# Enhex/RGK

Hardware: AMD Instinct MI355X
Metric: Mpaths/s, Sponza 1920x1080x256spp (path-tracing hot path) (higher is better)
Workload: dtype f32; 1 GPU; sponza-1080p 1920x1080x256spp depth 2 russian 0.74, strong scaling; geometry=proxy, triangles=64536, sampler=halton-cp, textures=handed over as u8; 0 of 0 float textures stored as bytes + value table, tiles=2040, parallelism=tiles round-robin over 1 GPU(s) + one RCCL reduce per round

## Files before the change

include/rgk.h:

```cpp
#ifndef RGK_H
#define RGK_H

#include <stdint.h>

#ifdef __cplusplus
extern "C" {
#endif

typedef enum rgk_status {
    RGK_OK = 0,
    RGK_ERR_INVALID = -1,
    RGK_ERR_DEVICE = -2,
    RGK_ERR_OOM = -3,
    RGK_ERR_NO_DEVICE = -4,
    RGK_ERR_UNSUPPORTED = -5
} rgk_status;

typedef enum rgk_bxdf_kind {
    RGK_BXDF_DIFFUSE = 0,
    RGK_BXDF_MIRROR = 1,
    RGK_BXDF_DIELECTRIC = 2,
    RGK_BXDF_TRANSPARENT = 3,
    RGK_BXDF_MIX = 4,
    RGK_BXDF_LTC_BECKMANN = 5,
// ... 97 lines not shown
typedef enum rgk_sampler_kind {
    RGK_SAMPLER_HALTON = 0,
    RGK_SAMPLER_STRATIFIED = 1
} rgk_sampler_kind;

#define RGK_FLAG_COUNT_TRAVERSAL 1u
#define RGK_FLAG_TIME_KERNELS 2u

typedef struct rgk_params {
    uint32_t xres, yres;
    uint32_t multisample;
    uint32_t depth;
    float clamp;
    float russian;
    float bumpmap_scale;
    uint32_t force_fresnell;
    uint32_t reverse;
    uint32_t sampler;
    uint32_t flags;
} rgk_params;

typedef struct rgk_tile {
    uint32_t x0, x1, y0, y1;
    uint32_t seed;
} rgk_tile;

typedef enum rgk_kernel_id {
    RGK_K_TRACE_CAMERA = 0,
    RGK_K_TRACE_CLOSEST,
    RGK_K_SHADE_FIRST,
    RGK_K_SHADE,
    RGK_K_SHADOW_FIRST,
    RGK_K_SHADOW,
    RGK_K_SHADOW_JOBS,
    RGK_K_CONNECT,
    RGK_K_LIGHT_TRACE,
    RGK_K_LIGHT_SHADE,
    RGK_K_LIGHT_SPLAT,
    RGK_K_RESOLVE,
    RGK_K_OTHER,
    RGK_K_COUNT
} rgk_kernel_id;

typedef struct rgk_kernel_stat {
    double ms;
    uint32_t launches;
    uint32_t reserved;
    uint64_t units;
    uint64_t node_visits;
    uint64_t tri_tests;
} rgk_kernel_stat;

typedef struct rgk_counters {
    uint64_t paths;
    uint64_t path_rays;
    uint64_t shadow_rays;
    uint64_t node_visits;
    uint64_t tri_tests;
    uint64_t shadow_node_visits;
    uint64_t shadow_tri_tests;
    double ms_trace;
    double ms_shadow;
    double ms_shade;
    double ms_other;
    uint32_t n_trace_launches;
    uint32_t n_shadow_launches;
    uint32_t n_shade_launches;
    uint32_t reserved;
    rgk_kernel_stat kernel[RGK_K_COUNT];
} rgk_counters;

typedef struct rgk_scene_info {
    float epsilon;
    float bbox_min[3];
    float bbox_max[3];
    float total_areal_power, total_point_power;
    uint32_t n_nodes;
    uint32_t node_bytes;
    uint32_t tri_bytes;
    uint32_t max_depth;
    uint32_t n_leaf_refs;
    uint32_t n_float_textures;
    uint32_t n_palettized_textures;
} rgk_scene_info;

typedef struct rgk_hit {
    float t;
    int32_t tri;
    float a, b, c;
} rgk_hit;

typedef struct rgk_progress {
    uint32_t stage, stages;
    uint32_t rounds;
    uint32_t busy;
    uint64_t round_pixels;
    uint64_t round_paths;
} rgk_progress;

typedef struct rgk_scene rgk_scene;

const char *rgk_last_error(void);
int rgk_device_count(void);

int rgk_scene_create(const rgk_scene_desc *desc, int device, rgk_scene **out);
int rgk_scene_refit(rgk_scene *scene, const float *vertices, const float *normals, const float *tangents);
void rgk_scene_destroy(rgk_scene *scene);
int rgk_scene_get_info(const rgk_scene *scene, rgk_scene_info *out);

int rgk_scene_get_progress(const rgk_scene *scene, rgk_progress *out);

int rgk_scene_set_tuning(rgk_scene *scene, const char *key, double value);

int rgk_generate_task_list(uint32_t tile_size, uint32_t xres, uint32_t yres, float mid_x,
                           float mid_y, uint32_t seedstart, uint32_t seedcount_base,
                           rgk_tile *tiles, uint32_t *n_tiles);

int rgk_camera_init(rgk_camera *out, const float pos[3], const float lookat[3], const float up[3], float yview,
                    float xview, int32_t xsize, int32_t ysize, float focus_plane, float lens_size);

int rgk_render_round(rgk_scene *scene, const rgk_camera *camera, const rgk_params *params,
                     const rgk_tile *tiles, uint32_t n_tiles, float *accum_rgb,
                     uint32_t *accum_count, rgk_counters *counters);

int rgk_render_round_device(rgk_scene *scene, const rgk_camera *camera,
                            const rgk_params *params, const rgk_tile *tiles, uint32_t n_tiles,
                            float *d_accum_rgb, uint32_t *d_accum_count,
                            rgk_counters *counters);

typedef struct rgk_accum rgk_accum;
int rgk_accum_create(uint32_t xres, uint32_t yres, int device, rgk_accum **out);
void rgk_accum_destroy(rgk_accum *acc);
int rgk_accum_clear(rgk_accum *acc);
float *rgk_accum_rgb(rgk_accum *acc);
uint32_t *rgk_accum_count(rgk_accum *acc);
int rgk_accum_download(const rgk_accum *acc, float *rgb, uint32_t *count);
int rgk_accum_upload(rgk_accum *acc, const float *rgb, const uint32_t *count);
int rgk_accum_add(rgk_accum *dst, const rgk_accum *src);
int rgk_accum_set_tag(rgk_accum *acc, uint64_t tag);

int rgk_accum_save(const rgk_accum *acc, const char *path, uint32_t rounds_done, uint32_t seedcount);
int rgk_accum_load(rgk_accum *acc, const char *path, uint32_t *rounds_done, uint32_t *seedcount);

typedef struct rgk_comm rgk_comm;
#define RGK_COMM_ID_BYTES 128
int rgk_shard_tiles(const rgk_tile *tiles, uint32_t n_tiles, int rank, int world_size, rgk_tile *out, uint32_t *n_out);
int rgk_comm_get_unique_id(uint8_t id[RGK_COMM_ID_BYTES]);
int rgk_comm_create(const uint8_t id[RGK_COMM_ID_BYTES], int rank, int world_size, int device, rgk_comm **out);
void rgk_comm_destroy(rgk_comm *comm);
int rgk_accum_reduce(rgk_comm *comm, float *d_accum_rgb, uint32_t *d_accum_count, uint32_t xres, uint32_t yres, int root);

int rgk_trace_closest(rgk_scene *scene, uint32_t n, const float *rays, const int32_t *ignore,
                      rgk_hit *hits, rgk_counters *counters);

int rgk_trace_visibility(rgk_scene *scene, uint32_t n, const float *a, const float *b,
                         uint8_t *visible, rgk_counters *counters);

int rgk_bxdf_value(rgk_scene *scene, uint32_t n, uint32_t route, const uint32_t *mat, const float *Vi, const float *Vr,
                   const float *uv, float *out_rgb);
int rgk_bxdf_sample(rgk_scene *scene, uint32_t n, uint32_t route, const uint32_t *mat, const float *Vi, const float *uv,
                    const float *u, float *out_dir, float *out_weight, uint8_t *may_leak);
int rgk_texture_sample(rgk_scene *scene, uint32_t n, const int32_t *tex, const float *uv, float *rgb, float *slope_right,
                       float *slope_bottom);

int rgk_libm_eval(int fn, uint32_t n, const float *a, const float *b, float *out);

// ... 16 lines not shown
```

rgk_amd/capi.py:

```python
import ctypes as C
import os

HERE = os.path.dirname(os.path.abspath(__file__))
LIB_PATH = os.environ.get("RGK_LIB") or os.path.join(HERE, "csrc", "librgk_hip.so")

BXDF_DIFFUSE, BXDF_MIRROR, BXDF_DIELECTRIC, BXDF_TRANSPARENT, BXDF_MIX = 0, 1, 2, 3, 4
BXDF_LTC_BECKMANN, BXDF_LTC_GGX, BXDF_LTC_BECKMANN_DIFFUSE, BXDF_LTC_GGX_DIFFUSE = 5, 6, 7, 8
MAT_NO_RUSSIAN = 1
TEX_SOLID, TEX_RGB32F, TEX_RGB8 = 0, 1, 2
SKY_COLOR, SKY_ENVMAP = 0, 1
SAMPLER_HALTON, SAMPLER_STRATIFIED = 0, 1
FLAG_COUNT_TRAVERSAL, FLAG_TIME_KERNELS = 1, 2
BUILD_AUTO, BUILD_DEVICE, BUILD_KEEP_FLOAT_TEXTURES, BUILD_HOST_SAH = 0, 1, 2, 4

BRDF_IDS = {
    "diffusecosine": BXDF_DIFFUSE, "diffuse": BXDF_DIFFUSE, "mix": BXDF_MIX,
    "dielectric": BXDF_DIELECTRIC, "mirror": BXDF_MIRROR, "transparent": BXDF_TRANSPARENT,
    "ltc_beckmann": BXDF_LTC_BECKMANN, "ltc_ggx": BXDF_LTC_GGX,
    "ltc_beckmann_diffuse": BXDF_LTC_BECKMANN_DIFFUSE, "ltc_ggx_diffuse": BXDF_LTC_GGX_DIFFUSE,
}

f3 = C.c_float * 3


class Material(C.Structure):
    _fields_ = [("kind", C.c_uint32), ("flags", C.c_uint32), ("emission", f3),
                ("roughness", C.c_float), ("ior", C.c_float), ("amount", C.c_float),
                ("tex_diffuse", C.c_int32), ("tex_color", C.c_int32), ("tex_bump", C.c_int32),
                ("mix_m1", C.c_int32), ("mix_m2", C.c_int32)]


class Texture(C.Structure):
    _fields_ = [("kind", C.c_uint32), ("width", C.c_uint32), ("height", C.c_uint32),
                ("color", f3), ("texels", C.POINTER(C.c_float)), ("texels8", C.POINTER(C.c_uint8)),
                ("lut", C.POINTER(C.c_float))]


class PointLight(C.Structure):
    _fields_ = [("pos", f3), ("color", f3), ("intensity", C.c_float), ("size", C.c_float)]


class SceneDesc(C.Structure):
    _fields_ = [("n_vertices", C.c_uint32),
                ("vertices", C.POINTER(C.c_float)), ("normals", C.POINTER(C.c_float)),
                ("tangents", C.POINTER(C.c_float)), ("texcoords", C.POINTER(C.c_float)),
                ("n_triangles", C.c_uint32),
                ("tri_indices", C.POINTER(C.c_uint32)), ("tri_material", C.POINTER(C.c_uint32)),
                ("n_materials", C.c_uint32), ("materials", C.POINTER(Material)),
                ("n_textures", C.c_uint32), ("textures", C.POINTER(Texture)),
                ("n_pointlights", C.c_uint32), ("pointlights", C.POINTER(PointLight)),
                ("n_areal_lights", C.c_uint32),
                ("areal_offsets", C.POINTER(C.c_uint32)), ("areal_tris", C.POINTER(C.c_uint32)),
                ("sky_mode", C.c_uint32), ("sky_color", f3), ("sky_intensity", C.c_float),
                ("sky_rotate", C.c_float), ("sky_texture", C.c_int32),
                ("ltc_ggx", C.POINTER(C.c_float)), ("ltc_beckmann", C.POINTER(C.c_float)), ("build_flags", C.c_uint32)]


class Camera(C.Structure):
    _fields_ = [("origin", f3), ("direction", f3), ("cameraup", f3), ("cameraleft", f3),
                ("viewscreen", f3), ("viewscreen_x", f3), ("viewscreen_y", f3),
                ("lens_size", C.c_float), ("xsize", C.c_int32), ("ysize", C.c_int32)]


class Params(C.Structure):
    _fields_ = [("xres", C.c_uint32), ("yres", C.c_uint32), ("multisample", C.c_uint32),
                ("depth", C.c_uint32), ("clamp", C.c_float), ("russian", C.c_float),
                ("bumpmap_scale", C.c_float), ("force_fresnell", C.c_uint32),
                ("reverse", C.c_uint32), ("sampler", C.c_uint32), ("flags", C.c_uint32)]


class Tile(C.Structure):
    _fields_ = [("x0", C.c_uint32), ("x1", C.c_uint32), ("y0", C.c_uint32), ("y1", C.c_uint32),
                ("seed", C.c_uint32)]


KERNEL_IDS = ["trace_camera", "trace_closest", "shade_first", "shade", "shadow_first", "shadow", "shadow_jobs", "connect",
              "light_trace", "light_shade", "light_splat", "resolve", "other"]
KERNEL_NAMES = {"trace_camera": "k_trace_camera", "trace_closest": "k_trace_closest", "shade_first": "k_shade<false, true", "shade": "k_shade<false, false",
                "shadow_first": "k_trace_shadow_first", "shadow": "k_trace_shadow<", "shadow_jobs": "k_trace_shadow_jobs", "connect": "k_connect",
                "resolve": "k_resolve"}


class KernelStat(C.Structure):
    _fields_ = [("ms", C.c_double), ("launches", C.c_uint32), ("reserved", C.c_uint32), ("units", C.c_uint64),
                ("node_visits", C.c_uint64), ("tri_tests", C.c_uint64)]


class Counters(C.Structure):
    _fields_ = [("paths", C.c_uint64), ("path_rays", C.c_uint64), ("shadow_rays", C.c_uint64),
                ("node_visits", C.c_uint64), ("tri_tests", C.c_uint64),
                ("shadow_node_visits", C.c_uint64), ("shadow_tri_tests", C.c_uint64),
                ("ms_trace", C.c_double), ("ms_shadow", C.c_double), ("ms_shade", C.c_double),
                ("ms_other", C.c_double), ("n_trace_launches", C.c_uint32),
                ("n_shadow_launches", C.c_uint32), ("n_shade_launches", C.c_uint32),
                ("reserved", C.c_uint32), ("kernel", KernelStat * len(KERNEL_IDS))]

    def as_dict(self):
        return {k: getattr(self, k) for k, _ in self._fields_ if k not in ("reserved", "kernel")}


class SceneInfo(C.Structure):
    _fields_ = [("epsilon", C.c_float), ("bbox_min", f3), ("bbox_max", f3),
                ("total_areal_power", C.c_float), ("total_point_power", C.c_float),
                ("n_nodes", C.c_uint32), ("node_bytes", C.c_uint32), ("tri_bytes", C.c_uint32),
                ("max_depth", C.c_uint32), ("n_leaf_refs", C.c_uint32),
                ("n_float_textures", C.c_uint32), ("n_palettized_textures", C.c_uint32)]


class Progress(C.Structure):
    _fields_ = [("stage", C.c_uint32), ("stages", C.c_uint32), ("rounds", C.c_uint32), ("busy", C.c_uint32),
                ("round_pixels", C.c_uint64), ("round_paths", C.c_uint64)]


class Hit(C.Structure):
    _fields_ = [("t", C.c_float), ("tri", C.c_int32), ("a", C.c_float), ("b", C.c_float),
                ("c", C.c_float)]


EXPORTS = ["rgk_last_error", "rgk_device_count", "rgk_scene_create", "rgk_scene_destroy",
           "rgk_scene_get_info", "rgk_scene_get_progress", "rgk_scene_set_tuning", "rgk_scene_refit", "rgk_generate_task_list", "rgk_camera_init", "rgk_render_round",
           "rgk_render_round_device", "rgk_trace_closest", "rgk_trace_visibility",
           "rgk_bxdf_value", "rgk_bxdf_sample", "rgk_texture_sample",
           "rgk_libm_eval", "rgk_sampler_eval", "rgk_output_normalize", "rgk_output_write_exr", "rgk_float_to_half",
           "rgk_accum_create", "rgk_accum_destroy", "rgk_accum_clear", "rgk_accum_rgb", "rgk_accum_count",
           "rgk_accum_download", "rgk_accum_upload", "rgk_accum_add", "rgk_accum_set_tag", "rgk_accum_save", "rgk_accum_load",
           "rgk_shard_tiles", "rgk_comm_get_unique_id", "rgk_comm_create", "rgk_comm_destroy", "rgk_accum_reduce"]

_p = C.POINTER


def _bind(lib):
    lib.rgk_last_error.restype = C.c_char_p
    lib.rgk_device_count.restype = C.c_int
    lib.rgk_scene_create.argtypes = [_p(SceneDesc), C.c_int, _p(C.c_void_p)]
    lib.rgk_scene_destroy.argtypes = [C.c_void_p]
    lib.rgk_scene_destroy.restype = None
    lib.rgk_scene_get_info.argtypes = [C.c_void_p, _p(SceneInfo)]
    lib.rgk_scene_get_progress.argtypes = [C.c_void_p, _p(Progress)]
    lib.rgk_scene_set_tuning.argtypes = [C.c_void_p, C.c_char_p, C.c_double]
    lib.rgk_scene_refit.argtypes = [C.c_void_p, C.c_void_p, C.c_void_p, C.c_void_p]
    lib.rgk_generate_task_list.argtypes = [C.c_uint32, C.c_uint32, C.c_uint32, C.c_float, C.c_float,
                                           C.c_uint32, C.c_uint32, _p(Tile), _p(C.c_uint32)]
    lib.rgk_camera_init.argtypes = [_p(Camera), f3, f3, f3, C.c_float, C.c_float, C.c_int32, C.c_int32, C.c_float, C.c_float]
    lib.rgk_render_round.argtypes = [C.c_void_p, _p(Camera), _p(Params), _p(Tile), C.c_uint32,
                                     C.c_void_p, C.c_void_p, _p(Counters)]
    lib.rgk_render_round_device.argtypes = lib.rgk_render_round.argtypes
    lib.rgk_trace_closest.argtypes = [C.c_void_p, C.c_uint32, C.c_void_p, C.c_void_p, C.c_void_p,
                                      _p(Counters)]
    lib.rgk_trace_visibility.argtypes = [C.c_void_p, C.c_uint32, C.c_void_p, C.c_void_p,
                                         C.c_void_p, _p(Counters)]
    lib.rgk_bxdf_value.argtypes = [C.c_void_p, C.c_uint32, C.c_uint32, C.c_void_p, C.c_void_p, C.c_void_p, C.c_void_p, C.c_void_p]
    lib.rgk_bxdf_sample.argtypes = [C.c_void_p, C.c_uint32, C.c_uint32, C.c_void_p, C.c_void_p, C.c_void_p, C.c_void_p, C.c_void_p, C.c_void_p, C.c_void_p]
    lib.rgk_texture_sample.argtypes = [C.c_void_p, C.c_uint32, C.c_void_p, C.c_void_p, C.c_void_p, C.c_void_p, C.c_void_p]
    lib.rgk_libm_eval.argtypes = [C.c_int, C.c_uint32, C.c_void_p, C.c_void_p, C.c_void_p]
    lib.rgk_sampler_eval.argtypes = [C.c_uint32, C.c_void_p, C.c_void_p, C.c_void_p, C.c_int,
                                     C.c_void_p]
    lib.rgk_output_normalize.argtypes = [C.c_void_p, C.c_void_p, C.c_uint32, C.c_uint32, C.c_float, C.c_void_p, _p(C.c_float)]
    lib.rgk_output_write_exr.argtypes = [C.c_char_p, C.c_uint32, C.c_uint32, C.c_void_p]
    lib.rgk_accum_create.argtypes = [C.c_uint32, C.c_uint32, C.c_int, _p(C.c_void_p)]
    lib.rgk_accum_destroy.argtypes = [C.c_void_p]
    lib.rgk_accum_destroy.restype = None
    lib.rgk_accum_clear.argtypes = [C.c_void_p]
    lib.rgk_accum_rgb.argtypes = [C.c_void_p]
    lib.rgk_accum_rgb.restype = C.c_void_p
    lib.rgk_accum_count.argtypes = [C.c_void_p]
    lib.rgk_accum_count.restype = C.c_void_p
    lib.rgk_accum_download.argtypes = [C.c_void_p, C.c_void_p, C.c_void_p]
    lib.rgk_accum_upload.argtypes = [C.c_void_p, C.c_void_p, C.c_void_p]
    lib.rgk_accum_add.argtypes = [C.c_void_p, C.c_void_p]
    lib.rgk_accum_set_tag.argtypes = [C.c_void_p, C.c_uint64]
    lib.rgk_accum_save.argtypes = [C.c_void_p, C.c_char_p, C.c_uint32, C.c_uint32]
    lib.rgk_accum_load.argtypes = [C.c_void_p, C.c_char_p, _p(C.c_uint32), _p(C.c_uint32)]
    lib.rgk_shard_tiles.argtypes = [_p(Tile), C.c_uint32, C.c_int, C.c_int, _p(Tile), _p(C.c_uint32)]
    lib.rgk_comm_get_unique_id.argtypes = [C.c_void_p]
    lib.rgk_comm_create.argtypes = [C.c_void_p, C.c_int, C.c_int, C.c_int, _p(C.c_void_p)]
    lib.rgk_comm_destroy.argtypes = [C.c_void_p]
    lib.rgk_comm_destroy.restype = None
    lib.rgk_accum_reduce.argtypes = [C.c_void_p, C.c_void_p, C.c_void_p, C.c_uint32, C.c_uint32, C.c_int]
    lib.rgk_float_to_half.argtypes = [C.c_float]
    lib.rgk_float_to_half.restype = C.c_uint16
    return lib


_product = None


def load_product():
    global _product
    if _product is None:
# ... 22 lines not shown
```

rgk_amd/csrc/device_types.h:

```cpp
#pragma once
#include <stdint.h>
#include <hip/hip_runtime.h>
#include "../../include/rgk.h"

#define RGK_NODE_BYTES 64
#define RGK_TRI_BYTES 48
#define RGK_LTC_TABLE_BYTES (4096u * 32u)

struct BvhNode {
    float lmin[3], lmax[3];
    float rmin[3], rmax[3];
    int32_t left, right;
    int32_t pad[2];
};

#define RGK_QNODE_EMPTY 0x7fffffff
struct QNode {
    float p[3];
    float sx;
    int32_t child[4];
    uint8_t qlo[3][4];
    uint8_t qhi[3][4];
    float sy, sz;
};
// ... 9 lines not shown

struct TriShade {
    float q[6][4];
    uint32_t mat, pad[7];
};

#define RGK_TEXREF_NONE 0xffffffffu
#ifndef RGK_TEX_TILED
#define RGK_TEX_TILED 1
#endif
struct TexRef {
    uint32_t kind, a, b, c;
};

struct DevMaterial {
    uint32_t kind, flags;
    float roughness, ior;
    float emission[3];
    float amount;
    int32_t mix_m1, mix_m2;
    int32_t pad[2];
    TexRef t_diffuse, t_color, t_bump;
};

struct DevPointLight {
    float pos[3];
    float intensity;
    float color[3];
    float size;
};

struct DevArealLight {
    float power;
    float total_area;
    float emission[3];
    uint32_t first, count;
    uint32_t pad;
};

struct DevArealTri {
    float area;
    uint32_t tri;
    float a[3], b[3], c[3];
    float normal_a[3];
    uint32_t light;
    uint32_t pad;
};

struct DevHaltonDim {
    uint32_t base;
    uint32_t digits;
    uint32_t perm_off;
    float scale;
    uint32_t magic;
    uint32_t shift;
    uint32_t pad[2];
};

struct DevCamera {
    float origin[3], direction[3], up[3], left[3];
    float viewscreen[3], viewscreen_x[3], viewscreen_y[3];
    float lens_size;
    int32_t xsize, ysize;
};

struct DevScene {
    const DevScene* self;
    const QNode* nodes;
    const TriIsect* tris;
    const TriShade* tri_shade;
    const DevMaterial* materials;
    const float4* texels;
    const uint32_t* texels8;
    const float* luts;
    uint32_t n_lut_floats, n_materials;
    const DevPointLight* pointlights;
    const DevArealLight* areal;
    const DevArealTri* areal_tris;
    const float4* ltc;
    const DevHaltonDim* hdims;
    const uint16_t* hperm;
    uint32_t n_pointlights, n_areal;
    float total_point_power, total_areal_power;
    float epsilon;
    float bb_min[3], bb_max[3];
    uint32_t has_texcoords;
    uint32_t walk_q;
    uint32_t sky_mode;
    float sky_color[3];
    float sky_intensity, sky_rotate;
    TexRef sky_tex;
};
```

rgk_amd/csrc/rgk_device.h:

```cpp
#pragma once
#include <hip/hip_runtime.h>
#include "device_types.h"
#include "../../include/rgk_libm.h"

#define RGK_PI_F 3.14159265358979323846264338327950288f

#define RGK_GLOBAL __attribute__((address_space(1)))
typedef float rgk_f4v __attribute__((ext_vector_type(4)));
__device__ __forceinline__ const RGK_GLOBAL char* gld_addr(const void* base, uint32_t byte_off) {
    const RGK_GLOBAL char* p = (const RGK_GLOBAL char*)base + byte_off;
    return p;
}
__device__ __forceinline__ uint32_t gld_u32(const void* base, uint32_t byte_off) { return *reinterpret_cast<const RGK_GLOBAL uint32_t*>(gld_addr(base, byte_off)); }
__device__ __forceinline__ uint32_t gld_u16(const void* base, uint32_t byte_off) { return *reinterpret_cast<const RGK_GLOBAL uint16_t*>(gld_addr(base, byte_off)); }
__device__ __forceinline__ float gld_f32(const void* base, uint32_t byte_off) { return *reinterpret_cast<const RGK_GLOBAL float*>(gld_addr(base, byte_off)); }
__device__ __forceinline__ float4 gld_f4(const void* base, uint32_t byte_off) {
    const rgk_f4v v = *reinterpret_cast<const RGK_GLOBAL rgk_f4v*>(gld_addr(base, byte_off));
    return make_float4(v.x, v.y, v.z, v.w);
}
template <typename T>
__device__ __forceinline__ T gld_rec(const void* base, uint32_t byte_off) {
    static_assert(sizeof(T) % 4 == 0, "record size");
    T out;
    uint32_t* o = reinterpret_cast<uint32_t*>(&out);
// ... 607 lines not shown
    float total_power = sc.total_point_power + sc.total_areal_power;
    if (total_power <= 0.0f) return L;
    float q = choice.x * total_power;
    if (q < sc.total_point_power) {
        for (uint32_t i = 0; i < sc.n_pointlights; i++) {
            const DevPointLight pl = gld_rec<DevPointLight>(sc.pointlights, i * (uint32_t)sizeof(DevPointLight));
            q -= pl.intensity * 4.0f * RGK_PI_F;
            if (q <= 0.0f) {
                L.type = 0;
                L.pos = mk3(pl.pos[0], pl.pos[1], pl.pos[2]);
                L.color = mk3(pl.color[0], pl.color[1], pl.color[2]);
                L.intensity = pl.intensity; L.size = pl.size; L.index = (int)i;
                return L;
            }
        }
        return L;
    }
    q = choice.y * sc.total_areal_power;
    for (uint32_t i = 0; i < sc.n_areal; i++) {
        const DevArealLight al = gld_rec<DevArealLight>(sc.areal, i * (uint32_t)sizeof(DevArealLight));
        q -= al.power;
        if (q <= 0.0f) {
            float p = light_sample * al.total_area;
            for (uint32_t j = 0; j < al.count; j++) {
                const DevArealTri att = gld_rec<DevArealTri>(sc.areal_tris, (al.first + j) * (uint32_t)sizeof(DevArealTri));
                const DevArealTri* at = &att;
                p -= at->area;
                if (p <= 0.0f) {
                    float2 r = tri_sample;
                    f3 a = mk3(at->a[0], at->a[1], at->a[2]);
                    f3 c = mk3(at->b[0], at->b[1], at->b[2]);
                    f3 b = mk3(at->c[0], at->c[1], at->c[2]);
                    f3 Va = a - c, Vb = b - c;
                    if (r.x + r.y > 1.0f) { r.x = 1.0f - r.x; r.y = 1.0f - r.y; }
                    L.type = 1;
                    L.pos = c + r.x * Va + r.y * Vb;
                    L.color = mk3(al.emission[0], al.emission[1], al.emission[2]);
                    L.intensity = 1.0f;
                    L.normal = mk3(at->normal_a[0], at->normal_a[1], at->normal_a[2]);
                    L.index = (int)(al.first + j);
                    return L;
                }
            }
            return L;
        }
    }
    return L;
}
#define RGK_LIGHT_NONE 0x7fffffffu
__device__ __forceinline__ uint32_t light_code(const DevScene& sc, float2 choice, float light_sample, float2 tri_sample, f3& pos) {
    DLight L = random_light(sc, choice, light_sample, tri_sample);
    pos = L.pos;
    if (L.type < 0) return RGK_LIGHT_NONE;
    if (L.type == 0) {
        pos = L.pos + L.size * sphere_uniform(tri_sample);
        return (uint32_t)L.index;
    }
    return 0x80000000u | (uint32_t)L.index;
}
__device__ __forceinline__ DLight light_from_code(const DevScene& sc, f3 pos, uint32_t code) {
    DLight L;
    L.pos = pos;
    L.normal = L.color = mk3(0.f, 0.f, 0.f);
    L.intensity = 0.f; L.size = 0.f; L.index = 0;
    if (code == RGK_LIGHT_NONE) { L.type = -1; return L; }
    if (code & 0x80000000u) {
        const DevArealTri att = gld_rec<DevArealTri>(sc.areal_tris, (code & 0x7fffffffu) * (uint32_t)sizeof(DevArealTri));
        const DevArealLight all = gld_rec<DevArealLight>(sc.areal, att.light * (uint32_t)sizeof(DevArealLight));
        const DevArealTri* at = &att;
        const DevArealLight* al = &all;
        L.type = 1;
        L.color = mk3(al->emission[0], al->emission[1], al->emission[2]);
        L.intensity = 1.0f;
        L.normal = mk3(at->normal_a[0], at->normal_a[1], at->normal_a[2]);
        return L;
    }
    const DevPointLight plv = gld_rec<DevPointLight>(sc.pointlights, code * (uint32_t)sizeof(DevPointLight));
    const DevPointLight* pl = &plv;
    L.type = 0;
    L.color = mk3(pl->color[0], pl->color[1], pl->color[2]);
    L.intensity = pl->intensity; L.size = pl->size;
    return L;
}
__device__ __forceinline__ f3 skybox(const DevScene& sc, f3 direction) {
    if (sc.sky_mode == 0) return mk3(sc.sky_color[0], sc.sky_color[1], sc.sky_color[2]) * mk3(sc.sky_intensity, sc.sky_intensity, sc.sky_intensity);
    float alpha = rgk_asinf(direction.y);
    float beta = -rgk_atan2f(direction.x, direction.z);
    beta += sc.sky_rotate * 0.0174533f;
    float x = beta / (2.0f * RGK_PI_F) + 0.5f;
    float y = alpha / RGK_PI_F + 0.5f;
    f3 c = tex_get(sc, sc.sky_tex, make_float2(x, y));
    return c * mk3(sc.sky_intensity, sc.sky_intensity, sc.sky_intensity);
}

struct Vertex {
    bool ok;
    f3 pos, faceN, lightN, Vr, VrL;
    float2 uv;
    uint32_t mat_id;
    DevMaterial mat;
    quatf g2l;
};
__device__ __forceinline__ f3 clamp3(f3 v, float c) { return mk3(v.x > c ? c : v.x, v.y > c ? c : v.y, v.z > c ? c : v.z); }

__device__ __forceinline__ void surface_point(const DevScene& sc, float bumpmap_scale, f3 o, f3 d, float4 h, Vertex& v) {
    const int tri = __float_as_int(h.w);
    const uint32_t tsr = (uint32_t)tri * (uint32_t)sizeof(TriShade);
    const float4 g0 = gld_f4(sc.tri_shade, tsr), g1 = gld_f4(sc.tri_shade, tsr + 16u), g2 = gld_f4(sc.tri_shade, tsr + 32u);
    v.mat_id = gld_u32(sc.tri_shade, tsr + 96u);
    v.mat = mat_load(sc, v.mat_id);
    const float al = h.y, be = h.z;
    const float ia = 1.0f - al - be, ib = al, ic = be;
    v.Vr = -d;
    v.pos = o + h.x * d;
    f3 nA_ = mk3(g0.x, g0.y, g0.z), nB_ = mk3(g1.x, g1.y, g1.z), nC_ = mk3(g2.x, g2.y, g2.z);
    f3 faceN = ia * nA_ + ib * nB_ + ic * nC_;
    v.ok = true;
    if (faceN.x != faceN.x) {
        faceN = nA_;
        if (faceN.x != faceN.x) { faceN = nB_; if (faceN.x != faceN.x) { faceN = nC_; if (faceN.x != faceN.x) v.ok = false; } }
    }
    if (v.ok && len3(faceN) <= 0.0f) v.ok = false;
    v.uv = make_float2(0.f, 0.f);
    v.faceN = v.lightN = faceN;
    if (!v.ok) return;
    faceN = norm3(faceN);
    const float4 g3 = gld_f4(sc.tri_shade, tsr + 48u), g4 = gld_f4(sc.tri_shade, tsr + 64u), g5 = gld_f4(sc.tri_shade, tsr + 80u);
    if (sc.has_texcoords) {
        v.uv.x = ia * g0.w + ib * g2.w + ic * g4.w;
        v.uv.y = ia * g1.w + ib * g3.w + ic * g5.w;
    }
    f3 lightN = faceN;
    if (tex_kind(v.mat.t_bump) != RGK_TEXREF_NONE) {
        float right, bottom;
        tex_slopes(sc, v.mat.t_bump, v.uv, right, bottom);
        f3 tangent = ia * mk3(g3.x, g3.y, g3.z) + ib * mk3(g4.x, g4.y, g4.z) + ic * mk3(g5.x, g5.y, g5.z);
        if (!(tangent.x * tangent.x + tangent.y * tangent.y + tangent.z * tangent.z < 0.001f)) {
            tangent = norm3(tangent);
            f3 bitangent = norm3(cross3(faceN, tangent));
            f3 tangent2 = cross3(bitangent, faceN);
            lightN = norm3(faceN + (tangent2 * right + bitangent * bottom) * bumpmap_scale);
            if (lightN.x != lightN.x) lightN = faceN;
        }
    }
    v.faceN = faceN;
    v.lightN = lightN;
    v.g2l = rotation_between(lightN, mk3(0.f, 0.f, 1.f));
    v.VrL = qrot(v.g2l, v.Vr);
}

__device__ __forceinline__ bool coords_from_direction(const DevCamera& cam, f3 dir, int& x, int& y) {
    const f3 N = mk3(cam.direction[0], cam.direction[1], cam.direction[2]);
    const f3 origin = mk3(cam.origin[0], cam.origin[1], cam.origin[2]);
    const f3 V = mk3(cam.viewscreen[0], cam.viewscreen[1], cam.viewscreen[2]);
    const f3 v1 = mk3(cam.viewscreen_x[0], cam.viewscreen_x[1], cam.viewscreen_x[2]);
    const f3 v2 = mk3(cam.viewscreen_y[0], cam.viewscreen_y[1], cam.viewscreen_y[2]);
    float q = dot3(dir, N);
    if ((double)q < 0.0001) return false;
    float t = dot3(V - origin, N) / q;
    if (t <= 0) return false;
    f3 p = origin + dir * t;
    f3 vp = p - V;
    float plen = len3(vp);
    float v1_cast_len = plen * (dot3(norm3(vp), norm3(v1)));
    float v2_cast_len = plen * (dot3(norm3(vp), norm3(v2)));
    float x_ratio = v1_cast_len / len3(v1);
// ... 9 lines not shown
```

rgk_amd/csrc/rgk_host.cpp:

```cpp
#include <hip/hip_runtime.h>

#include <algorithm>
#include <array>
#include <iterator>
#include <atomic>
#include <cmath>
#include <cstdarg>
#include <cstdio>
#include <cstdlib>
#include <cstring>
#include <limits>
#include <string>
#include <vector>
#include <functional>
#include <random>

#include "../../include/rgk.h"
#include "device_types.h"
#include "rgk_kernels.h"
#include "rgk_build.h"

namespace {

thread_local std::string g_err;
// ... 347 lines not shown
        Box nb;
        nb.reset();
        for (auto& c : ch) nb.grow(c.box);
        QNode q;
        std::memset(&q, 0, sizeof(q));
        for (int a = 0; a < 3; a++) {
            q.p[a] = nb.mn[a];
            float ext = nb.mx[a] - nb.mn[a];
            int e = 0;
            if (ext > 0.f) { std::frexp(ext / 255.0f, &e); } else e = -126;
            for (;; e++) {
                if (e < -126) e = -126;
                const float scale = std::ldexp(1.0f, e);
                bool ok = true;
                uint8_t lo[4], hi[4];
                for (size_t i = 0; i < ch.size() && ok; i++) {
                    float fl = std::floor((ch[i].box.mn[a] - q.p[a]) / scale), fh = std::ceil((ch[i].box.mx[a] - q.p[a]) / scale);
                    if (fl < 0.f) fl = 0.f;
                    while (fl > 0.f && std::fmaf(fl, scale, q.p[a]) > ch[i].box.mn[a]) fl -= 1.f;
                    while (fh <= 255.f && std::fmaf(fh, scale, q.p[a]) < ch[i].box.mx[a]) fh += 1.f;
                    if (fh > 255.f || fl > 255.f) { ok = false; break; }
                    lo[i] = (uint8_t)fl; hi[i] = (uint8_t)fh;
                }
                if (!ok) continue;
                (a == 0 ? q.sx : (a == 1 ? q.sy : q.sz)) = scale;
                for (size_t i = 0; i < 4; i++) { q.qlo[a][i] = i < ch.size() ? lo[i] : 255; q.qhi[a][i] = i < ch.size() ? hi[i] : 0; }
                break;
            }
        }
        for (size_t i = 0; i < 4; i++) q.child[i] = RGK_QNODE_EMPTY;
        out[idx] = q;
        for (size_t i = 0; i < ch.size(); i++) {
            int ref = ch[i].ref;
            if (ref >= 0) ref = collapse(ref, depth + 1, stack_before + pushed);
            out[idx].child[i] = ref;
        }
        return idx;
    }
};

template <typename T>
struct DevBuf {
    T* p = nullptr;
    size_t n = 0;
    DevBuf() = default;
    DevBuf(const DevBuf&) = delete;
    DevBuf& operator=(const DevBuf&) = delete;
    ~DevBuf() { release(); }
    int alloc(size_t count) {
        if (count <= n && p) return 0;
        if (p) (void)hipFree(p);
        p = nullptr; n = 0;
        if (count == 0) count = 1;
        hipError_t e = hipMalloc((void**)&p, count * sizeof(T));
        if (e != hipSuccess) return fail(RGK_ERR_OOM, "hipMalloc(%zu bytes): %s", count * sizeof(T), hipGetErrorString(e));
        n = count;
        static const bool poison = std::getenv("RGK_POISON") != nullptr;
        if (poison) {
            (void)hipMemset(p, 0xFF, count * sizeof(T));
            (void)hipDeviceSynchronize();
        }
        return 0;
    }
    int upload(const T* src, size_t count) {
        int rc = alloc(count);
        if (rc) return rc;
        if (count) {
            hipError_t e = hipMemcpy(p, src, count * sizeof(T), hipMemcpyHostToDevice);
            if (e != hipSuccess) return fail(RGK_ERR_DEVICE, "hipMemcpy H2D: %s", hipGetErrorString(e));
        }
        return 0;
    }
    void release() { if (p) (void)hipFree(p); p = nullptr; n = 0; }
};

}

extern "C" __attribute__((visibility("hidden"))) int rgk_internal_fail(int code, const char* msg) { return fail(code, "%s", msg); }

struct RgkTuning {
    bool entry_points = true;
    bool entry_cap = true;
    bool light_entry = true;
    int sample_group = -1;
    size_t batch_paths = 0;
    double workspace_gb = 0;
    int beam = 1;
    bool debug_bvh = false, debug_util = false;
};

struct rgk_scene {
    int device = 0;
    RgkTuning tune;
    hipStream_t stream = nullptr;
    rgk_scene_info info{};
    DevScene dev{};
    RgkTraceCfg tcfg{32, 32, nullptr};
    DevBuf<int> ovf;
    DevBuf<QNode> nodes;
    DevBuf<TriIsect> tris;
    DevBuf<TriShade> tri_shade;
    DevBuf<DevMaterial> materials;
    DevBuf<float4> texels;
    DevBuf<uint32_t> texels8;
    DevBuf<float> luts;
    DevBuf<DevPointLight> pointlights;
    DevBuf<DevArealLight> areal;
    DevBuf<DevArealTri> areal_tris;
    DevBuf<float4> ltc;
    DevBuf<DevScene> self;
    DevBuf<uint32_t> generic;
    DevBuf<TexRef> texrefs;
    DevBuf<uint32_t> d_idx;
    DevBuf<float4> leaf_pb;
    std::vector<uint32_t> h_idx, h_tri_mat, h_areal_off, h_areal_tris;
    std::vector<rgk_material> h_mats;
    std::vector<float> h_normals;
    uint32_t n_vertices = 0, n_triangles = 0, n_refs = 0, n_nodes = 0;
    uint32_t n_textures = 0, n_materials = 0;
    DevBuf<DevHaltonDim> hdims;
    DevBuf<uint16_t> hperm;
    size_t batch = 0;
    DevBuf<float4> rayA[2], rayB[2], hit, thr, tot, shA, shB, shC, pixsum, light;
    DevBuf<float4> lstart, lv;
    DevBuf<uint32_t> hitlist;
    DevBuf<uint32_t> lvmask, connlist;
    DevBuf<float4> conn, jobs, rads;
    uint32_t batch_reverse = 0;
    DevBuf<float> htab;
    DevBuf<float2> nearfar;
    DevBuf<uint32_t> counters, pix_xy, pix_seed, tile_buf;
    DevBuf<int> entry;
    DevBuf<float> entry_cap;
    size_t entry_capped = 0;
    DevBuf<int> lentry;
    DevBuf<uint32_t> trange;
    DevBuf<float4> lbox;
    size_t lentry_done = 0;
    uint64_t entry_key = 0;
    size_t entry_n = 0;
    DevBuf<unsigned long long> stats;
    DevBuf<float> scratch_f;
    DevBuf<uint32_t> scratch_u;
    std::vector<hipEvent_t> events;
    uint32_t* h_counters = nullptr;
    std::atomic<uint32_t> prog_stages{0}, prog_rounds{0}, prog_busy{0};
    uint32_t* h_stage = nullptr;
    std::atomic<uint64_t> prog_pixels{0}, prog_paths{0};
    ~rgk_scene() {
        (void)hipSetDevice(device);
        if (stream) (void)hipStreamSynchronize(stream);
        for (auto e : events) (void)hipEventDestroy(e);
        if (h_counters) (void)hipHostFree(h_counters);
        if (h_stage) (void)hipHostFree(h_stage);
        if (stream) (void)hipStreamDestroy(stream);
    }
};

namespace {

int ensure_workspace(rgk_scene* s, size_t paths, uint32_t reverse = 0) {
    if (paths <= s->batch && reverse <= s->batch_reverse) return 0;
    if (s->batch) { paths = std::max(paths, s->batch); reverse = std::max(reverse, s->batch_reverse); }
    int rc = 0;
    for (int i = 0; i < 2 && !rc; i++) { rc = s->rayA[i].alloc(paths); if (!rc) rc = s->rayB[i].alloc(paths); }
    if (!rc) rc = s->hit.alloc(paths);
    if (!rc) rc = s->thr.alloc(paths);
    if (!rc) rc = s->tot.alloc(paths);
    if (!rc) rc = s->shA.alloc(paths);
    if (!rc) rc = s->shB.alloc(paths);
    if (!rc) rc = s->shC.alloc(paths);
    if (reverse) {
        if (!rc) rc = s->lstart.alloc(paths);
        if (!rc) rc = s->lv.alloc(paths * RGK_LV_FLOAT4 * reverse);
        if (!rc) rc = s->hitlist.alloc(paths);
        if (!rc) rc = s->lvmask.alloc(paths);
        if (!rc) rc = s->connlist.alloc(paths);
        if (!rc) rc = s->conn.alloc(paths * 6);
        if (!rc) rc = s->jobs.alloc(paths * 4);
        if (!rc) rc = s->rads.alloc(paths * ((size_t)reverse + 1));
    }
    if (!rc) rc = s->light.alloc(paths);
    if (!rc) rc = s->generic.alloc(paths);
    if (!rc) rc = s->counters.alloc(2 * RGK_CNT_TOTAL);
    if (!rc) rc = s->stats.alloc(8);
    if (rc) { s->batch = 0; s->batch_reverse = 0; return rc; }
    if (!s->h_counters) HIPCHK(hipHostMalloc((void**)&s->h_counters, 2 * RGK_CNT_TOTAL * sizeof(uint32_t)));
    if (!s->h_stage) { HIPCHK(hipHostMalloc((void**)&s->h_stage, sizeof(uint32_t))); *s->h_stage = 0; }
    s->batch = paths;
// ... 131 lines not shown
        std::fprintf(stderr, "[rgk desc] material %u kind %u flags %u emission %g %g %g rough %.9g ior %.9g amount %.9g tex %d %d %d mix %d %d\n", i, m.kind, m.flags, m.emission[0], m.emission[1],
                     m.emission[2], m.roughness, m.ior, m.amount, m.tex_diffuse, m.tex_color, m.tex_bump, m.mix_m1, m.mix_m2);
    }
    for (uint32_t i = 0; i < d->n_textures; i++) {
        const rgk_texture& t = d->textures[i];
        const size_t n = (size_t)t.width * t.height;
        std::fprintf(stderr, "[rgk desc] texture %u kind %u %ux%u color %.9g %.9g %.9g texels %016llx\n", i, t.kind, t.width, t.height, t.color[0], t.color[1], t.color[2],
                     t.kind == RGK_TEX_RGB32F ? h(t.texels, 12 * n) : (t.kind == RGK_TEX_RGB8 ? h(t.texels8, 3 * n) ^ h(t.lut, 1024) : 0ull));
    }
    std::fprintf(stderr, "[rgk desc] pointlights %u %016llx areal %u offsets %016llx tris %016llx\n", d->n_pointlights, h(d->pointlights, sizeof(rgk_pointlight) * (size_t)d->n_pointlights),
                 d->n_areal_lights, h(d->areal_offsets, 4ull * (d->n_areal_lights + 1)), h(d->areal_tris, d->n_areal_lights ? 4ull * d->areal_offsets[d->n_areal_lights] : 0));
    std::fprintf(stderr, "[rgk desc] sky mode %u color %.9g %.9g %.9g intensity %.9g rotate %.9g tex %d ltc %016llx %016llx\n", d->sky_mode, d->sky_color[0], d->sky_color[1], d->sky_color[2],
                 d->sky_intensity, d->sky_rotate, d->sky_texture, h(d->ltc_ggx, 4096 * 20), h(d->ltc_beckmann, 4096 * 20));
}

#ifndef RGK_SAMPLE_GROUP_DEFAULT
#define RGK_SAMPLE_GROUP_DEFAULT 3
#endif
static void build_areal_tables(const float* vertices, const float* normals, const uint32_t* tri_indices, const uint32_t* tri_material, const rgk_material* materials,
                               uint32_t n_areal, const uint32_t* areal_offsets, const uint32_t* areal_tris, std::vector<DevArealLight>& als,
                               std::vector<DevArealTri>& ats, float& total_areal) {
    auto vert = [&](uint32_t i) { return V3{vertices[3 * i], vertices[3 * i + 1], vertices[3 * i + 2]}; };
    als.clear(); ats.clear(); total_areal = 0.f;
    for (uint32_t i = 0; i < n_areal; i++) {
        uint32_t b = areal_offsets[i], e = areal_offsets[i + 1];
        if (e <= b) continue;
        std::vector<std::pair<float, uint32_t>> twa;
        float total_area = 0.f;
        for (uint32_t j = b; j < e; j++) {
            uint32_t t = areal_tris[j];
            V3 A = vert(tri_indices[3 * t]), B = vert(tri_indices[3 * t + 1]), C = vert(tri_indices[3 * t + 2]);
            V3 c = crossv(sub(A, B), sub(C, B));
            float area = 0.5f * std::sqrt(dotv(c, c));
            twa.push_back({area, t});
            total_area += area;
        }
        const rgk_material& m0 = materials[tri_material[twa[0].second]];
        std::sort(twa.rbegin(), twa.rend());
        DevArealLight al{};
        al.total_area = total_area;
        for (int k = 0; k < 3; k++) al.emission[k] = m0.emission[k];
        al.power = total_area * (m0.emission[0] + m0.emission[1] + m0.emission[2]);
        al.first = (uint32_t)ats.size();
        al.count = (uint32_t)twa.size();
        for (auto& p : twa) {
            DevArealTri at{};
            at.area = p.first; at.tri = p.second; at.light = (uint32_t)als.size();
            uint32_t ia = tri_indices[3 * p.second], ib = tri_indices[3 * p.second + 1], ic = tri_indices[3 * p.second + 2];
            for (int k = 0; k < 3; k++) {
                at.a[k] = vertices[3 * ia + k]; at.b[k] = vertices[3 * ib + k]; at.c[k] = vertices[3 * ic + k];
                at.normal_a[k] = normals[3 * ia + k];
            }
            ats.push_back(at);
        }
        total_areal += al.power;
        als.push_back(al);
    }
}

#ifndef RGK_BUILD_AUTO_DEVICE_REFS
#define RGK_BUILD_AUTO_DEVICE_REFS 500000
#endif
#ifndef RGK_LBVH_ROTATE_PASSES
#define RGK_LBVH_ROTATE_PASSES 4
#endif
int rgk_scene_create(const rgk_scene_desc* d, int device, rgk_scene** out) {
    if (!out) return fail(RGK_ERR_INVALID, "null output pointer");
    *out = nullptr;
    int rc = validate_desc(d);
    if (rc) return rc;
    if (std::getenv("RGK_DEBUG_DESC")) debug_desc(d);
    int ndev = 0;
    if (hipGetDeviceCount(&ndev) != hipSuccess || ndev == 0) return fail(RGK_ERR_NO_DEVICE, "no HIP device visible");
    if (device < 0 || device >= ndev) return fail(RGK_ERR_INVALID, "device %d out of range (%d visible)", device, ndev);
    HIPCHK(hipSetDevice(device));
    rgk_scene* s = new rgk_scene;
    s->device = device;
    struct Guard { rgk_scene* s; ~Guard() { delete s; } } guard{s};
    HIPCHK(hipStreamCreateWithFlags(&s->stream, hipStreamNonBlocking));
    {
        auto off = [](const char* name) { const char* e = std::getenv(name); return e && e[0] == '0'; };
        RgkTuning& t = s->tune;
        t.entry_points = !off("RGK_ENTRY_POINTS"); t.entry_cap = !off("RGK_ENTRY_CAP"); t.light_entry = !off("RGK_LIGHT_ENTRY");
        if (const char* e = std::getenv("RGK_SAMPLE_GROUP")) t.sample_group = std::min(6, std::max(0, std::atoi(e)));
        if (const char* e = std::getenv("RGK_BATCH_PATHS")) t.batch_paths = std::max<size_t>(1024, strtoull(e, nullptr, 10));
        if (const char* e = std::getenv("RGK_WORKSPACE_GB")) t.workspace_gb = atof(e);
        if (const char* e = std::getenv("RGK_BEAM")) t.beam = std::min(2, std::max(0, std::atoi(e)));
        t.debug_bvh = std::getenv("RGK_DEBUG_BVH") != nullptr; t.debug_util = std::getenv("RGK_DEBUG_UTIL") != nullptr;
    }

    const uint32_t nt = d->n_triangles;
    auto vert = [&](uint32_t i) { return V3{d->vertices[3 * i], d->vertices[3 * i + 1], d->vertices[3 * i + 2]}; };

    float mn[3], mx[3];
    for (int a = 0; a < 3; a++) { mn[a] = std::numeric_limits<float>::infinity(); mx[a] = -mn[a]; }
    for (uint32_t i = 0; i < nt; i++)
        for (int k = 0; k < 3; k++) {
            V3 v = vert(d->tri_indices[3 * i + k]);
            for (int a = 0; a < 3; a++) { float c = comp(v, a); if (c < mn[a]) mn[a] = c; if (c > mx[a]) mx[a] = c; }
        }
    float xs = mx[0] - mn[0], ys = mx[1] - mn[1], zs = mx[2] - mn[2];
    float diameter = std::sqrt(xs * xs + ys * ys + zs * zs);
    float eps = 0.00001f * diameter;
    if (!(eps == eps) || !(diameter < std::numeric_limits<float>::infinity())) return fail(RGK_ERR_INVALID, "non-finite vertex coordinates");
    DevScene& ds = s->dev;
    ds.epsilon = eps;
    for (int a = 0; a < 3; a++) { ds.bb_min[a] = mn[a] - eps; ds.bb_max[a] = mx[a] + eps; }

    std::vector<TriIsect> recs(nt);
    std::vector<Prim> prims;
    prims.reserve(nt);
    RefSplitter splitter;
    {
        const char* e = std::getenv("RGK_BVH_SPLIT");
        const float f = e ? (float)std::atof(e) : 0.1f;
        splitter.lmax = f > 0.f ? f * (eps * 1e5f) : 0.f;
        splitter.budget = (size_t)nt;
        splitter.out = &prims;
    }
    for (uint32_t i = 0; i < nt; i++) {
        V3 v0 = vert(d->tri_indices[3 * i]), v1 = vert(d->tri_indices[3 * i + 1]), v2 = vert(d->tri_indices[3 * i + 2]);
        V3 d0 = sub(v1, v0), d1 = sub(v2, v0);
        V3 n = normv(crossv(d1, d0));
        float dd = -dotv(n, v0);
        TriIsect& r = recs[i];
        r.n[0] = n.x; r.n[1] = n.y; r.n[2] = n.z; r.d = dd;
        int i1, i2;
        float ax = std::fabs(n.x), ay = std::fabs(n.y), az = std::fabs(n.z);
        if (ax > ay && ax > az) { i1 = 1; i2 = 2; }
        else if (ay > az) { i1 = 0; i2 = 2; }
        else { i1 = 0; i2 = 1; }
        r.v0a = comp(v0, i1); r.v0b = comp(v0, i2);
        r.q1x = comp(v1, i1) - comp(v0, i1); r.q1y = comp(v1, i2) - comp(v0, i2);
        r.q2x = comp(v2, i1) - comp(v0, i1); r.q2y = comp(v2, i2) - comp(v0, i2);
        r.axes = (uint32_t)i1 | ((uint32_t)i2 << 2);
        r.tri = i;
        if (n.x == n.x && n.y == n.y && n.z == n.z) {
            Prim p;
            for (int a = 0; a < 3; a++) {
                p.bmin[a] = std::min(comp(v0, a), std::min(comp(v1, a), comp(v2, a)));
                p.bmax[a] = std::max(comp(v0, a), std::max(comp(v1, a), comp(v2, a)));
                p.c[a] = 0.5f * (p.bmin[a] + p.bmax[a]);
            }
            p.tri = i;
            p.pb[0] = 0.f; p.pb[1] = 1.f; p.pb[2] = 0.f; p.pb[3] = 1.f;
            if (splitter.lmax > 0.f) {
                std::vector<RefSplitter::P3> poly(3);
                for (int a = 0; a < 3; a++) { poly[0].x[a] = comp(v0, a); poly[1].x[a] = comp(v1, a); poly[2].x[a] = comp(v2, a); }
                for (int c = 0; c < 3; c++) for (int a = 0; a < 3; a++) splitter.tv[c][a] = poly[c].x[a];
                splitter.emit(poly, p.bmin, p.bmax, i, 0);
            } else {
                p.ref = (uint32_t)prims.size();
                prims.push_back(p);
            }
        }
    }
    if (prims.empty()) return fail(RGK_ERR_INVALID, "every triangle is degenerate");
    if (prims.size() >= (1u << 25)) return fail(RGK_ERR_UNSUPPORTED, "too many triangles (32-bit byte offsets into the triangle tables: < 2^25)");
    std::vector<QNode> qnodes;
    std::vector<TriIsect> leaf_recs;
    std::vector<float4> leaf_pb;
    std::vector<uint32_t> ref_tri(prims.size());
    std::vector<float4> ref_pb(prims.size());
    for (const Prim& p : prims) { ref_tri[p.ref] = p.tri; ref_pb[p.ref] = make_float4(p.pb[0], p.pb[1], p.pb[2], p.pb[3]); }
    uint32_t max_depth = 0, max_stack = 0, n_nodes = 0, n_refs = (uint32_t)prims.size();
    bool on_device = false;
// ... 174 lines not shown
                for (size_t k = 0; k < n; k++)
                    put(k, index_of(t.texels[3 * k]) | (index_of(t.texels[3 * k + 1]) << 8) | (index_of(t.texels[3 * k + 2]) << 16));
            }
        } else {
            n_float_tex++;
            if (t.width > 65535 || t.height > 65535) return fail(RGK_ERR_UNSUPPORTED, "texture %u larger than 65535 texels on a side", i);
            const size_t n = (size_t)t.width * t.height;
            if (pool.size() + n >= (1ull << 28)) return fail(RGK_ERR_UNSUPPORTED, "float texel pool exceeds 2^28 texels");
            o.a = t.width | (t.height << 16);
            o.b = (uint32_t)pool.size();
            pool.reserve(pool.size() + n);
            for (size_t k = 0; k < n; k++) pool.push_back(make_float4(t.texels[3 * k], t.texels[3 * k + 1], t.texels[3 * k + 2], 0.f));
        }
    }
    auto tref = [&](int32_t id) { TexRef r; r.kind = RGK_TEXREF_NONE; r.a = r.b = r.c = 0; return id < 0 ? r : trefs[id]; };
    std::vector<DevMaterial> mats(d->n_materials);
    for (uint32_t i = 0; i < d->n_materials; i++) {
        const rgk_material& m = d->materials[i];
        DevMaterial& o = mats[i];
        std::memset(&o, 0, sizeof(o));
        o.kind = m.kind; o.flags = m.flags;
        for (int k = 0; k < 3; k++) o.emission[k] = m.emission[k];
        o.roughness = m.roughness; o.ior = m.ior; o.amount = m.amount;
        o.t_diffuse = tref(m.tex_diffuse); o.t_color = tref(m.tex_color); o.t_bump = tref(m.tex_bump);
        o.mix_m1 = m.mix_m1; o.mix_m2 = m.mix_m2;
    }
    std::vector<DevPointLight> pls(d->n_pointlights);
    float total_point = 0.f;
    const float PI_F = 3.14159265358979323846264338327950288f;
    for (uint32_t i = 0; i < d->n_pointlights; i++) {
        const rgk_pointlight& l = d->pointlights[i];
        DevPointLight& o = pls[i];
        for (int k = 0; k < 3; k++) { o.pos[k] = l.pos[k]; o.color[k] = l.color[k]; }
        o.intensity = l.intensity; o.size = l.size;
        total_point += l.intensity * 4.0f * PI_F;
    }
    std::vector<DevArealLight> als;
    std::vector<DevArealTri> ats;
    float total_areal = 0.f;
    build_areal_tables(d->vertices, d->normals, d->tri_indices, d->tri_material, d->materials, d->n_areal_lights, d->areal_offsets, d->areal_tris, als, ats, total_areal);
    std::vector<DevHaltonDim> hd;
    std::vector<uint16_t> hp;
    build_halton(hd, hp);

    s->n_textures = d->n_textures; s->n_materials = d->n_materials;
    s->n_vertices = d->n_vertices; s->n_triangles = nt; s->n_refs = n_refs; s->n_nodes = n_nodes;
    s->h_idx.assign(d->tri_indices, d->tri_indices + 3 * (size_t)nt);
    s->h_tri_mat.assign(d->tri_material, d->tri_material + nt);
    s->h_mats.assign(d->materials, d->materials + d->n_materials);
    s->h_normals.assign(d->normals, d->normals + 3 * (size_t)d->n_vertices);
    if (d->n_areal_lights) {
        s->h_areal_off.assign(d->areal_offsets, d->areal_offsets + d->n_areal_lights + 1);
        s->h_areal_tris.assign(d->areal_tris, d->areal_tris + d->areal_offsets[d->n_areal_lights]);
    }
    if ((rc = s->d_idx.upload(s->h_idx.data(), s->h_idx.size()))) return rc;
    if ((rc = s->texrefs.upload(trefs.data(), trefs.size()))) return rc;
    if (!on_device && ((rc = s->nodes.upload(qnodes.data(), qnodes.size())) || (rc = s->tris.upload(leaf_recs.data(), leaf_recs.size())) ||
                       (rc = s->leaf_pb.upload(leaf_pb.data(), leaf_pb.size()))))
        return rc;
    if ((rc = s->tri_shade.upload(tsh.data(), tsh.size())) ||
        (rc = s->materials.upload(mats.data(), mats.size())) || (rc = s->texels.upload(pool.data(), pool.size())) || (rc = s->texels8.upload(pool8.data(), pool8.size())) ||
        (rc = s->luts.upload(luts.data(), luts.size())) || (rc = s->pointlights.upload(pls.data(), pls.size())) || (rc = s->areal.upload(als.data(), als.size())) ||
        (rc = s->areal_tris.upload(ats.data(), ats.size())) || (rc = s->hdims.upload(hd.data(), hd.size())) || (rc = s->hperm.upload(hp.data(), hp.size())))
        return rc;
    {
        std::vector<float4> t(2 * 2 * 4096, make_float4(0.f, 0.f, 0.f, 0.f));
        const float* src[2] = {d->ltc_ggx, d->ltc_beckmann};
        for (int w = 0; w < 2; w++)
            for (int k = 0; src[w] && k < 4096; k++) {
                t[(size_t)w * 8192 + 2 * k] = make_float4(src[w][5 * k], src[w][5 * k + 1], src[w][5 * k + 2], src[w][5 * k + 3]);
                t[(size_t)w * 8192 + 2 * k + 1] = make_float4(src[w][5 * k + 4], 0.f, 0.f, 0.f);
            }
        if ((rc = s->ltc.upload(t.data(), t.size()))) return rc;
    }
    ds.nodes = s->nodes.p;
    { const char* e = std::getenv("RGK_WALK_Q"); ds.walk_q = e ? (uint32_t)std::atoi(e) : 3u; }
    if (s->tune.debug_bvh) std::fprintf(stderr, "[rgk] bvh4 (%s) nodes %u max_stack %u max_depth %u refs %u of %u triangles\n", on_device ? "device LBVH" : "host SAH", n_nodes, max_stack, max_depth, n_refs, nt);
    ds.tris = s->tris.p; ds.tri_shade = s->tri_shade.p;
    ds.materials = s->materials.p; ds.texels = s->texels.p; ds.texels8 = s->texels8.p; ds.luts = s->luts.p; ds.n_lut_floats = (uint32_t)luts.size(); ds.n_materials = (uint32_t)mats.size();
    ds.pointlights = s->pointlights.p; ds.areal = s->areal.p; ds.areal_tris = s->areal_tris.p;
    ds.ltc = s->ltc.p; ds.hdims = s->hdims.p; ds.hperm = s->hperm.p;
    ds.n_pointlights = (uint32_t)pls.size(); ds.n_areal = (uint32_t)als.size();
    ds.total_point_power = total_point; ds.total_areal_power = total_areal;
    ds.has_texcoords = d->texcoords ? 1u : 0u;
    ds.sky_mode = d->sky_mode;
    for (int k = 0; k < 3; k++) ds.sky_color[k] = d->sky_color[k];
    ds.sky_intensity = d->sky_intensity; ds.sky_rotate = d->sky_rotate; ds.sky_tex = tref(d->sky_mode == RGK_SKY_ENVMAP ? d->sky_texture : -1);
    if ((rc = s->self.alloc(1))) return rc;
    ds.self = s->self.p;
    if (hipMemcpy(s->self.p, &ds, sizeof(DevScene), hipMemcpyHostToDevice) != hipSuccess) return fail(RGK_ERR_DEVICE, "hipMemcpy(DevScene)");

    rgk_scene_info& inf = s->info;
    inf.epsilon = eps;
    for (int a = 0; a < 3; a++) { inf.bbox_min[a] = ds.bb_min[a]; inf.bbox_max[a] = ds.bb_max[a]; }
    inf.total_areal_power = total_areal; inf.total_point_power = total_point;
    inf.n_nodes = n_nodes; inf.node_bytes = RGK_NODE_BYTES; inf.tri_bytes = RGK_TRI_BYTES;
    inf.max_depth = max_depth; inf.n_leaf_refs = n_refs;
    inf.n_float_textures = n_float_tex; inf.n_palettized_textures = n_palettized;
    guard.s = nullptr;
    *out = s;
    return RGK_OK;
}

int rgk_scene_refit(rgk_scene* s, const float* vertices, const float* normals, const float* tangents) {
    if (!s || !vertices) return fail(RGK_ERR_INVALID, "null argument");
    if (s->prog_busy.load()) return fail(RGK_ERR_INVALID, "rgk_scene_refit while a round is in flight on this scene");
    HIPCHK(hipSetDevice(s->device));
    const uint32_t nt = s->n_triangles, nv = s->n_vertices;
    float mn[3], mx[3];
    for (int a = 0; a < 3; a++) { mn[a] = std::numeric_limits<float>::infinity(); mx[a] = -mn[a]; }
    for (size_t k = 0; k < 3 * (size_t)nt; k++) {
        const float* v = vertices + 3 * (size_t)s->h_idx[k];
        for (int a = 0; a < 3; a++) { if (v[a] < mn[a]) mn[a] = v[a]; if (v[a] > mx[a]) mx[a] = v[a]; }
    }
    const float xs = mx[0] - mn[0], ys = mx[1] - mn[1], zs = mx[2] - mn[2];
    const float diameter = std::sqrt(xs * xs + ys * ys + zs * zs);
    const float eps = 0.00001f * diameter;
    if (!(eps == eps) || !(diameter < std::numeric_limits<float>::infinity())) return fail(RGK_ERR_INVALID, "non-finite vertex coordinates");
    int rc;
    if ((rc = s->scratch_f.upload(vertices, 3 * (size_t)nv))) return rc;
    DevBuf<float> d_n, d_t;
    if (normals && (rc = d_n.upload(normals, 3 * (size_t)nv))) return rc;
    if (tangents && (rc = d_t.upload(tangents, 3 * (size_t)nv))) return rc;
    const char* err = "";
    rc = rgk_refit_bvh4_device(s->stream, s->n_refs, s->n_nodes, nt, s->scratch_f.p, normals ? d_n.p : nullptr, tangents ? d_t.p : nullptr, s->d_idx.p, s->leaf_pb.p, eps,
                               s->tris.p, s->nodes.p, s->tri_shade.p, &err);
    if (rc) return fail(rc, "refit: %s", err);
    if (normals) s->h_normals.assign(normals, normals + 3 * (size_t)nv);
    std::vector<DevArealLight> als;
    std::vector<DevArealTri> ats;
    float total_areal = 0.f;
    build_areal_tables(vertices, s->h_normals.data(), s->h_idx.data(), s->h_tri_mat.data(), s->h_mats.data(), (uint32_t)(s->h_areal_off.empty() ? 0 : s->h_areal_off.size() - 1),
                       s->h_areal_off.data(), s->h_areal_tris.data(), als, ats, total_areal);
    if ((rc = s->areal.upload(als.data(), als.size())) || (rc = s->areal_tris.upload(ats.data(), ats.size()))) return rc;
    DevScene& ds = s->dev;
    ds.areal = s->areal.p; ds.areal_tris = s->areal_tris.p; ds.n_areal = (uint32_t)als.size(); ds.total_areal_power = total_areal;
    ds.epsilon = eps;
    for (int a = 0; a < 3; a++) { ds.bb_min[a] = mn[a] - eps; ds.bb_max[a] = mx[a] + eps; }
    if (hipMemcpy(s->self.p, &ds, sizeof(DevScene), hipMemcpyHostToDevice) != hipSuccess) return fail(RGK_ERR_DEVICE, "hipMemcpy(DevScene)");
    s->info.epsilon = eps; s->info.total_areal_power = total_areal;
    for (int a = 0; a < 3; a++) { s->info.bbox_min[a] = ds.bb_min[a]; s->info.bbox_max[a] = ds.bb_max[a]; }
    s->entry_key = 0; s->entry_n = 0; s->entry_capped = 0; s->lentry_done = 0;
    return RGK_OK;
}

void rgk_scene_destroy(rgk_scene* s) { delete s; }

int rgk_scene_get_info(const rgk_scene* s, rgk_scene_info* out) {
    if (!s || !out) return fail(RGK_ERR_INVALID, "null argument");
    *out = s->info;
    return RGK_OK;
}

int rgk_scene_get_progress(const rgk_scene* s, rgk_progress* out) {
    if (!s || !out) return fail(RGK_ERR_INVALID, "null argument");
    out->stage = s->h_stage ? *(volatile const uint32_t*)s->h_stage : 0u; out->stages = s->prog_stages.load(); out->rounds = s->prog_rounds.load(); out->busy = s->prog_busy.load();
    out->round_pixels = s->prog_pixels.load(); out->round_paths = s->prog_paths.load();
    if (out->stage > out->stages) out->stage = out->stages;
    return RGK_OK;
}

int rgk_scene_set_tuning(rgk_scene* s, const char* key, double value) {
    if (!s || !key) return fail(RGK_ERR_INVALID, "null argument");
    if (s->prog_busy.load()) return fail(RGK_ERR_INVALID, "rgk_scene_set_tuning while a round is in flight on this scene");
    RgkTuning& t = s->tune;
    const std::string k(key);
    if (k == "entry_points") t.entry_points = value != 0;
    else if (k == "entry_cap") t.entry_cap = value != 0;
    else if (k == "light_entry") t.light_entry = value != 0;
    else if (k == "sample_group") t.sample_group = value < 0 ? -1 : (int)std::min(6.0, value);
    else if (k == "batch_paths") t.batch_paths = value <= 0 ? 0 : std::max<size_t>(1024, (size_t)value);
    else if (k == "workspace_gb") t.workspace_gb = value <= 0 ? 0.0 : value;
    else if (k == "beam") t.beam = (int)std::min(2.0, std::max(0.0, value));
    else return fail(RGK_ERR_INVALID, "unknown tuning key '%s'", key);
    s->entry_key = 0; s->entry_n = 0; s->entry_capped = 0; s->lentry_done = 0;
    return RGK_OK;
}

int rgk_generate_task_list(uint32_t tile_size, uint32_t xres, uint32_t yres, float mid_x, float mid_y, uint32_t seedstart,
                           uint32_t seedcount_base, rgk_tile* tiles, uint32_t* n_tiles) {
    if (!n_tiles || tile_size == 0) return fail(RGK_ERR_INVALID, "bad argument");
    struct T { rgk_tile t; float d; };
    std::vector<T> v;
    for (uint32_t yp = 0; yp < yres; yp += tile_size)
        for (uint32_t xp = 0; xp < xres; xp += tile_size) {
            T t;
            t.t.x0 = xp; t.t.x1 = std::min(xres, xp + tile_size);
            t.t.y0 = yp; t.t.y1 = std::min(yres, yp + tile_size);
            t.t.seed = 0;
            float mx = (t.t.x0 + t.t.x1) / 2.0f, my = (t.t.y0 + t.t.y1) / 2.0f;
            float dx = mid_x - mx, dy = mid_y - my;
            t.d = std::sqrt(dx * dx + dy * dy);
            v.push_back(t);
        }
    std::stable_sort(v.begin(), v.end(), [](const T& a, const T& b) { return a.d < b.d; });
    if (tiles) {
        if (*n_tiles < v.size()) return fail(RGK_ERR_INVALID, "tile buffer too small (%u < %zu)", *n_tiles, v.size());
        for (size_t i = 0; i < v.size(); i++) { tiles[i] = v[i].t; tiles[i].seed = seedstart + seedcount_base + (uint32_t)i; }
    }
    *n_tiles = (uint32_t)v.size();
    return RGK_OK;
}

int rgk_camera_init(rgk_camera* o, const float pos[3], const float lookat[3], const float upv[3], float yview, float xview, int32_t xsize,
                    int32_t ysize, float focus_plane, float lens_size) {
    if (!o || !pos || !lookat || !upv) return fail(RGK_ERR_INVALID, "null argument");
    V3 origin{pos[0], pos[1], pos[2]}, la{lookat[0], lookat[1], lookat[2]}, up{upv[0], upv[1], upv[2]};
    V3 direction = normv(sub(la, origin));
    V3 left = normv(crossv(up, direction));
    up = normv(crossv(left, direction));
    V3 vx = scale(scale(left, -xview), focus_plane);
    V3 vy = scale(scale(up, yview), focus_plane);
    V3 a = {origin.x + direction.x * focus_plane, origin.y + direction.y * focus_plane, origin.z + direction.z * focus_plane};
    V3 hy = scale(vy, 0.5f), hx = scale(vx, 0.5f);
    V3 vs = sub(sub(a, hy), hx);
    auto put = [](float* dst, V3 v) { dst[0] = v.x; dst[1] = v.y; dst[2] = v.z; };
    put(o->origin, origin); put(o->direction, direction); put(o->cameraup, up); put(o->cameraleft, left);
    put(o->viewscreen, vs); put(o->viewscreen_x, vx); put(o->viewscreen_y, vy);
    o->lens_size = lens_size; o->xsize = xsize; o->ysize = ysize;
    return RGK_OK;
}

static void make_camera(const rgk_camera* c, DevCamera& o) {
    for (int k = 0; k < 3; k++) {
        o.origin[k] = c->origin[k]; o.direction[k] = c->direction[k]; o.up[k] = c->cameraup[k]; o.left[k] = c->cameraleft[k];
        o.viewscreen[k] = c->viewscreen[k]; o.viewscreen_x[k] = c->viewscreen_x[k]; o.viewscreen_y[k] = c->viewscreen_y[k];
    }
    o.lens_size = c->lens_size; o.xsize = c->xsize; o.ysize = c->ysize;
}

static size_t batch_paths(const RgkTuning& tune, uint32_t reverse) {
    if (tune.batch_paths) return tune.batch_paths;
    const size_t per_path = 180 + (reverse ? 16 + 16 * RGK_LV_FLOAT4 * (size_t)reverse + 12 + 16 * (6 + 4 + (size_t)reverse + 1) : 0);
    const bool g = tune.workspace_gb > 0;
    double gb = g ? tune.workspace_gb : (reverse ? 160.0 : 96.0);
    if (!g) {
        size_t free_b = 0, total_b = 0;
        if (hipMemGetInfo(&free_b, &total_b) == hipSuccess && free_b > 0) gb = std::min(gb, 0.6 * (double)free_b / 1e9);
    }
    size_t b = (size_t)(gb * 1e9 / (double)per_path);
    return std::min<size_t>(std::max<size_t>(b, 1024), (size_t)1 << 30);
}

}

namespace {

struct KernelLog {
    rgk_scene* s;
    bool timing, count_stats;
    struct Ev { int cls; hipEvent_t a, b; };
    std::vector<Ev> evs;
// ... 97 lines not shown
    for (uint32_t i = 0; i < n_tiles; i++) {
        const rgk_tile& t = tiles[i];
        if (t.x1 > prm->xres || t.y1 > prm->yres || t.x0 > t.x1 || t.y0 > t.y1) return fail(RGK_ERR_INVALID, "tile %u outside the frame", i);
        const uint64_t n = (uint64_t)toff[i] + (uint64_t)(t.x1 - t.x0) * (t.y1 - t.y0);
        if (n >= (1ull << 31)) return fail(RGK_ERR_UNSUPPORTED, "more than 2^31 pixels in one round");
        toff[i + 1] = (uint32_t)n;
    }
    P = toff[n_tiles];
    if (P == 0) return 0;
    hipStream_t st = s->stream;
    int rc;
    if ((rc = s->pix_xy.alloc(P)) || (rc = s->pix_seed.alloc(P)) || (rc = s->tile_buf.alloc((size_t)n_tiles * 5 + n_tiles + 1))) return rc;
    static_assert(sizeof(rgk_tile) == 5 * sizeof(uint32_t), "rgk_tile layout");
    HIPCHK(hipMemcpyAsync(s->tile_buf.p, tiles, (size_t)n_tiles * sizeof(rgk_tile), hipMemcpyHostToDevice, st));
    HIPCHK(hipMemcpyAsync(s->tile_buf.p + (size_t)n_tiles * 5, toff.data(), (n_tiles + 1) * sizeof(uint32_t), hipMemcpyHostToDevice, st));
    rgk_launch_build_pixel_list(st, reinterpret_cast<const rgk_tile*>(s->tile_buf.p), s->tile_buf.p + (size_t)n_tiles * 5, n_tiles, s->pix_xy.p, s->pix_seed.p);
    if (!s->tune.entry_points) {
        s->entry.release(); s->entry_cap.release();
        return 0;
    }
    uint64_t key = 1469598103934665603ull;
    auto mix = [&key](const void* p, size_t n) { const unsigned char* b = (const unsigned char*)p; for (size_t i = 0; i < n; i++) { key ^= b[i]; key *= 1099511628211ull; } };
    mix(camera, sizeof(*camera)); mix(&prm->xres, sizeof(prm->xres)); mix(&prm->yres, sizeof(prm->yres));
    for (uint32_t t = 0; t < n_tiles; t++) mix(&tiles[t], 4 * sizeof(uint32_t));
    const size_t n_entry = ((size_t)P + RGK_ENTRY_PIX - 1) / RGK_ENTRY_PIX * RGK_ENTRY_K;
    if (s->entry.p && s->entry_n == n_entry && s->entry_key == key) return 0;
    if ((rc = s->entry.alloc(n_entry)) || (rc = s->entry_cap.alloc(n_entry / RGK_ENTRY_K + 1)) || (rc = s->trange.alloc((n_entry / RGK_ENTRY_K + 1) * 2))) return rc;
    DevCamera cam0;
    make_camera(camera, cam0);
    rgk_launch_entry_points(st, s->dev, cam0, prm->xres, prm->yres, s->pix_xy.p, (uint32_t)P, 0u, (uint32_t)(n_entry / RGK_ENTRY_K), nullptr, s->entry.p, s->entry_cap.p);
    s->entry_key = key; s->entry_n = n_entry;
    s->entry_capped = 0; s->lentry_done = 0;
    return 0;
}

int plan_passes(rgk_scene* s, const rgk_params* prm, size_t P, uint32_t R, size_t& npix_pass, uint32_t& ns_pass) {
    size_t B = batch_paths(s->tune, R);
    if (!s->tune.batch_paths && s->batch_reverse >= R) B = std::max(B, s->batch);
    int rc;
    for (;;) {
        npix_pass = std::min(P, B);
        const uint32_t ns_max = (uint32_t)std::max<size_t>(1, std::min<size_t>(prm->multisample, B / npix_pass));
        const uint32_t n_sample_passes = (prm->multisample + ns_max - 1) / ns_max;
        ns_pass = (prm->multisample + n_sample_passes - 1) / n_sample_passes;
        rc = ensure_workspace(s, npix_pass * ns_pass, R);
        if (rc != RGK_ERR_OOM || B <= ((size_t)1 << 20)) break;
        (void)hipGetLastError();
        B /= 2;
    }
    if (rc) return rc;
    return s->pixsum.alloc(P);
}

int queue_first_hit_lists(rgk_scene* s, KernelLog& kl, const DevCamera& cam, PassParams& pp, uint32_t P, bool cap_entries, bool light_entry) {
    hipStream_t st = s->stream;
    const size_t end = (size_t)pp.j0 + pp.npix;
    const bool need_cap = cap_entries && end > s->entry_capped;
    const bool need_light = light_entry && end > s->lentry_done;
    int rc;
    if ((need_cap || need_light) && (rc = kl.run(RGK_K_OTHER, [&] { rgk_launch_group_trange(st, pp, s->hit.p, s->trange.p); }))) return rc;
    if (need_cap) {
        const uint32_t g_first = pp.j0 >> RGK_ENTRY_SHIFT, g_last = (uint32_t)((end + RGK_ENTRY_PIX - 1) >> RGK_ENTRY_SHIFT);
        if ((rc = kl.run(RGK_K_OTHER, [&] { rgk_launch_entry_points(st, s->dev, cam, pp.xres, pp.yres, s->pix_xy.p, P, g_first, g_last - g_first, s->trange.p, s->entry.p, s->entry_cap.p); })))
            return rc;
        s->entry_capped = end;
    }
    if (!light_entry) return 0;
    pp.lentry = s->lentry.p; pp.lbox = s->lbox.p;
    if (!need_light) return 0;
    if ((rc = kl.run(RGK_K_OTHER, [&] { rgk_launch_light_entry_points(st, s->dev, cam, pp, P, s->trange.p, s->lentry.p, s->lbox.p); }))) return rc;
    s->lentry_done = end;
    if (s->tune.debug_bvh) {
        const size_t g0 = pp.j0 >> RGK_ENTRY_SHIFT, g1 = (end + RGK_ENTRY_PIX - 1) >> RGK_ENTRY_SHIFT;
        std::vector<int> he((g1 - g0) * RGK_ENTRY_K);
        HIPCHK(hipStreamSynchronize(st));
        HIPCHK(hipMemcpy(he.data(), s->lentry.p + g0 * RGK_ENTRY_K, he.size() * sizeof(int), hipMemcpyDeviceToHost));
        size_t below = 0, total_e = 0;
        for (size_t g = 0; g < g1 - g0; g++) { if (he[g * RGK_ENTRY_K] != 0) below++; for (int k = 0; k < RGK_ENTRY_K; k++) total_e += he[g * RGK_ENTRY_K + k] != 0x7fffffff; }
        std::fprintf(stderr, "[rgk] light-side entry nodes: %zu of %zu pixel groups start below the root, %.2f entries per group\n", below, g1 - g0, (double)total_e / (double)(g1 - g0));
    }
    return 0;
}

int queue_pass(rgk_scene* s, KernelLog& kl, const DevCamera& cam, PassParams& pp, size_t P, bool light_entry, float* d_accum_rgb,
               uint32_t* d_accum_count, uint32_t stage) {
    hipStream_t st = s->stream;
    const RgkTraceCfg& tc = s->tcfg;
    const bool count_stats = kl.count_stats, cap_entries = s->entry.p != nullptr && s->tune.entry_cap;
    const bool track = pp.depth > 12;
    const uint32_t R = pp.reverse, n0 = pp.npix * pp.ns;
    {
        uint32_t g = s->tune.sample_group >= 0 ? (uint32_t)s->tune.sample_group : (uint32_t)RGK_SAMPLE_GROUP_DEFAULT;
        while (g && (pp.ns & ((1u << g) - 1u))) g--;
        pp.gshift = g;
        const bool lists_capped = cap_entries && (size_t)pp.j0 + pp.npix <= s->entry_capped;
        pp.beam = (s->tune.beam == 2 || (s->tune.beam == 1 && !lists_capped)) ? 1u : 0u;
    }
    float4* const rayA[2] = {s->rayA[0].p, s->rayA[1].p};
    float4* const rayB[2] = {s->rayB[0].p, s->rayB[1].p};
    float4 *const hit = s->hit.p, *const thr = s->thr.p, *const tot = s->tot.p, *const shA = s->shA.p, *const shB = s->shB.p, *const shC = s->shC.p;
    uint32_t* const cn = s->counters.p;
    uint32_t* const cl = cn + RGK_CNT_TOTAL;
    int rc;
    if (R > 0) {
        rgk_launch_set_bound(n0, n0);
        if ((rc = kl.run(RGK_K_OTHER, [&] { rgk_launch_init_counters(st, cl, 0u); })) ||
            (rc = kl.run(RGK_K_LIGHT_SHADE, [&] { rgk_launch_raygen_light(st, s->dev, cam, pp, rayA[0], rayB[0], thr, cl); })))
            return rc;
        for (uint32_t k = 0; k < R; k++) {
            const int q = k & 1;
            if ((rc = kl.run(RGK_K_LIGHT_TRACE, [&] { rgk_launch_trace_closest(st, s->dev, tc, count_stats, rayA[q], rayB[q], nullptr, hit, cl + RGK_CNT_QUEUE + k, cl + RGK_CNT_FETCH_T + k, s->stats.p); })) ||
                (rc = kl.run(RGK_K_LIGHT_SHADE, [&] { rgk_launch_list_hits(st, hit, cl + RGK_CNT_QUEUE + k, s->hitlist.p, cl + RGK_CNT_HITS + k); })) ||
                (rc = kl.run(RGK_K_LIGHT_SHADE, [&] { rgk_launch_shade_light(st, s->dev, cam, pp, k, rayA[q], rayB[q], hit, thr, rayA[q ^ 1], rayB[q ^ 1], shA, shB, shC, cl); })) ||
                (rc = kl.run(RGK_K_LIGHT_SPLAT, [&] { rgk_launch_trace_shadow(st, s->dev, tc, count_stats, shA, shB, shC, nullptr, nullptr, RGK_SHADOW_SPLAT, d_accum_rgb,
                                                                              cl + RGK_CNT_SHADOW + k, cl + RGK_CNT_FETCH_S + k, s->stats.p); })))
                return rc;
        }
    }
    if ((rc = kl.run(RGK_K_OTHER, [&] { rgk_launch_init_counters(st, cn, n0); }))) return rc;
    uint32_t ub = n0;
    for (uint32_t b = 0; b < pp.depth && ub > 0; b++) {
        const int q = b & 1;
        rgk_launch_set_bound(ub, ub);
        if (b == 0)
            rc = kl.run(RGK_K_TRACE_CAMERA, [&] { rgk_launch_trace_camera(st, s->dev, cam, pp, tc, count_stats, hit, cn + RGK_CNT_QUEUE, cn + RGK_CNT_FETCH_T, s->stats.p); });
        else
            rc = kl.run(RGK_K_TRACE_CLOSEST, [&] { rgk_launch_trace_closest(st, s->dev, tc, count_stats, rayA[q], rayB[q], nullptr, hit, cn + RGK_CNT_QUEUE + b, cn + RGK_CNT_FETCH_T + b, s->stats.p); });
        if (rc || (b == 0 && (rc = queue_first_hit_lists(s, kl, cam, pp, (uint32_t)P, cap_entries, light_entry)))) return rc;
        if ((rc = kl.run(b == 0 ? RGK_K_SHADE_FIRST : RGK_K_SHADE, [&] { rgk_launch_shade(st, s->dev, cam, pp, b, rayA[q], rayB[q], hit, thr, tot, rayA[q ^ 1], rayB[q ^ 1], shA, shB, shC, cn, R > 0); })) ||
            (R > 0 && (rc = kl.run(RGK_K_CONNECT, [&] { rgk_launch_connect(st, s->dev, pp, b, s->jobs.p, s->rads.p, cn); }))))
            return rc;
        if (b == 0 && light_entry)
            rc = kl.run(RGK_K_SHADOW_FIRST, [&] { rgk_launch_trace_shadow_first(st, s->dev, pp, tc, count_stats, shA, shB, shC, tot, cn + RGK_CNT_SHADOW + b, cn + RGK_CNT_FETCH_S + b, s->stats.p); });
        else
            rc = kl.run(RGK_K_SHADOW, [&] { rgk_launch_trace_shadow(st, s->dev, tc, count_stats, shA, shB, shC, tot, nullptr, RGK_SHADOW_ADD, nullptr, cn + RGK_CNT_SHADOW + b, cn + RGK_CNT_FETCH_S + b, s->stats.p); });
        if (rc || (R > 0 && (rc = kl.run(RGK_K_SHADOW_JOBS, [&] { rgk_launch_trace_shadow_jobs(st, s->dev, pp, tc, count_stats, s->jobs.p, s->rads.p, tot, cn + RGK_CNT_CONN + b, cn + RGK_CNT_FETCH_J + b, s->stats.p); }))))
            return rc;
        rgk_launch_stage_mark(st, s->h_stage, stage + b + 1);
        if (track && b >= 3 && (b & 1) && b + 1 < pp.depth && (rc = queue_len(s, cn + RGK_CNT_QUEUE + b + 1, ub))) return rc;
    }
    if ((rc = kl.run(RGK_K_RESOLVE, [&] { rgk_launch_resolve(st, pp, tot, s->pixsum.p, d_accum_rgb, d_accum_count); }))) return rc;
    rgk_launch_stage_mark(st, s->h_stage, stage + std::max(1u, pp.depth));
    HIPCHK(hipMemcpyAsync(s->h_counters, cn, 2 * RGK_CNT_TOTAL * sizeof(uint32_t), hipMemcpyDeviceToHost, st));
    return 0;
}
}

extern "C" {

int rgk_render_round_device(rgk_scene* s, const rgk_camera* camera, const rgk_params* prm, const rgk_tile* tiles, uint32_t n_tiles,
                            float* d_accum_rgb, uint32_t* d_accum_count, rgk_counters* counters) {
    if (!s || !camera || !prm || (!tiles && n_tiles) || !d_accum_rgb || !d_accum_count) return fail(RGK_ERR_INVALID, "null argument");
    if (prm->xres == 0 || prm->yres == 0 || prm->xres > 65535 || prm->yres > 65535) return fail(RGK_ERR_INVALID, "resolution out of range");
    if (prm->multisample == 0) return fail(RGK_ERR_INVALID, "multisample must be >= 1");
    if (prm->depth > RGK_MAX_DEPTH) return fail(RGK_ERR_UNSUPPORTED, "recursion depth %u > %d", prm->depth, RGK_MAX_DEPTH);
    if (prm->reverse > 7) return fail(RGK_ERR_UNSUPPORTED, "reverse %u > 7 light sub-path vertices", prm->reverse);
    if (prm->sampler != RGK_SAMPLER_HALTON) return fail(RGK_ERR_UNSUPPORTED, "the HIP path implements the Halton sampler only");
    HIPCHK(hipSetDevice(s->device));
    if (counters) std::memset(counters, 0, sizeof(*counters));
    std::vector<uint32_t> toff;
    size_t P = 0, npix_pass = 0;
    uint32_t ns_pass = 0;
    int rc;
    if ((rc = prepare_round_lists(s, camera, prm, tiles, n_tiles, toff, P))) return rc;
    if (P == 0) return RGK_OK;
    const uint32_t R = (s->dev.total_point_power + s->dev.total_areal_power > 0.0f) ? prm->reverse : 0u;
    if ((rc = plan_passes(s, prm, P, R, npix_pass, ns_pass))) return rc;

    DevCamera cam;
    make_camera(camera, cam);
    HIPCHK(hipMemsetAsync(s->stats.p, 0, 8 * sizeof(unsigned long long), s->stream));
    KernelLog kl(s, prm->flags);
    const uint32_t pass_stages = std::max(1u, prm->depth);
    {
        const uint32_t n_pix_passes = (uint32_t)((P + npix_pass - 1) / npix_pass), n_s_passes = (prm->multisample + ns_pass - 1) / ns_pass;
        *(volatile uint32_t*)s->h_stage = 0; s->prog_stages = n_pix_passes * n_s_passes * pass_stages;
        s->prog_pixels = P; s->prog_paths = (uint64_t)P * prm->multisample; s->prog_busy = 1;
    }
    struct Done { rgk_scene* s; ~Done() { *(volatile uint32_t*)s->h_stage = s->prog_stages.load(); s->prog_busy = 0; } } done_guard{s};
    PassParams pp{};
    pp.multisample = prm->multisample; pp.depth = prm->depth; pp.xres = prm->xres; pp.yres = prm->yres;
    pp.clamp = prm->clamp; pp.russian = prm->russian; pp.bumpmap_scale = prm->bumpmap_scale; pp.reverse = R;
    pp.lstart = s->lstart.p; pp.lv = s->lv.p; pp.hitlist = s->hitlist.p; pp.lvmask = s->lvmask.p; pp.conn = s->conn.p; pp.connlist = s->connlist.p;
    pp.batch = (uint32_t)s->batch;
    pp.pix_xy = s->pix_xy.p; pp.pix_seed = s->pix_seed.p; pp.light = s->light.p; pp.generic = s->generic.p;
    pp.entry = s->entry.p;
    pp.entry_cap = s->entry_cap.p;
    const bool light_entry = s->entry.p && s->tune.light_entry && s->dev.n_pointlights == 1 && s->dev.n_areal == 0;
    if (light_entry) {
        const size_t groups = ((size_t)P + RGK_ENTRY_PIX - 1) / RGK_ENTRY_PIX + 1;
        if ((rc = s->lentry.alloc(groups * RGK_ENTRY_K)) || (rc = s->trange.alloc(groups * 2)) || (rc = s->lbox.alloc(groups * 2))) return rc;
    }
    if ((rc = s->htab.alloc((size_t)192 * prm->multisample))) return rc;
    if ((rc = kl.run(RGK_K_OTHER, [&] { rgk_launch_build_halton_table(s->stream, s->dev, prm->multisample, s->htab.p); }))) return rc;
    pp.htab = s->htab.p;

    rgk_counters tot{};
    uint32_t stage = 0;
    for (size_t j0 = 0; j0 < P; j0 += npix_pass) {
        pp.j0 = (uint32_t)j0;
        pp.npix = (uint32_t)std::min(npix_pass, P - j0);
        for (uint32_t s0 = 0; s0 < prm->multisample; s0 += ns_pass, stage += pass_stages) {
            pp.s0 = s0;
            pp.ns = std::min(ns_pass, prm->multisample - s0);
            if ((rc = queue_pass(s, kl, cam, pp, P, light_entry, d_accum_rgb, d_accum_count, stage))) return rc;
            HIPCHK(hipStreamSynchronize(s->stream));
            add_pass_counters(s->h_counters, pp, light_entry, tot);
        }
    }
    HIPCHK(hipGetLastError());
    s->prog_rounds++;
    if (counters) {
        tot.paths = (uint64_t)P * prm->multisample;
        if (kl.count_stats) {
            unsigned long long h[8];
            HIPCHK(hipMemcpy(h, s->stats.p, sizeof(h), hipMemcpyDeviceToHost));
            tot.node_visits = h[0]; tot.tri_tests = h[1]; tot.shadow_node_visits = h[2]; tot.shadow_tri_tests = h[3];
        }
        if ((rc = kl.fold(tot))) return rc;
        *counters = tot;
    }
    return RGK_OK;
}

int rgk_render_round(rgk_scene* s, const rgk_camera* camera, const rgk_params* prm, const rgk_tile* tiles, uint32_t n_tiles,
                     float* accum_rgb, uint32_t* accum_count, rgk_counters* counters) {
    if (!s || !prm || !accum_rgb || !accum_count) return fail(RGK_ERR_INVALID, "null argument");
    HIPCHK(hipSetDevice(s->device));
    const size_t P = (size_t)prm->xres * prm->yres;
    float* d_rgb = nullptr;
    uint32_t* d_cnt = nullptr;
    HIPCHK(hipMalloc((void**)&d_rgb, P * 3 * sizeof(float)));
    hipError_t e = hipMalloc((void**)&d_cnt, P * sizeof(uint32_t));
    if (e != hipSuccess) { (void)hipFree(d_rgb); return fail(RGK_ERR_OOM, "hipMalloc: %s", hipGetErrorString(e)); }
    int rc = RGK_OK;
    auto chk = [&](hipError_t x, const char* what) { if (x != hipSuccess && rc == RGK_OK) rc = fail(RGK_ERR_DEVICE, "%s: %s", what, hipGetErrorString(x)); };
    chk(hipMemcpy(d_rgb, accum_rgb, P * 3 * sizeof(float), hipMemcpyHostToDevice), "upload accumulator");
    chk(hipMemcpy(d_cnt, accum_count, P * sizeof(uint32_t), hipMemcpyHostToDevice), "upload counts");
    if (rc == RGK_OK) rc = rgk_render_round_device(s, camera, prm, tiles, n_tiles, d_rgb, d_cnt, counters);
    if (rc == RGK_OK) {
        chk(hipMemcpy(accum_rgb, d_rgb, P * 3 * sizeof(float), hipMemcpyDeviceToHost), "download accumulator");
        chk(hipMemcpy(accum_count, d_cnt, P * sizeof(uint32_t), hipMemcpyDeviceToHost), "download counts");
    }
    (void)hipFree(d_rgb);
    (void)hipFree(d_cnt);
    return rc;
}

int rgk_trace_closest(rgk_scene* s, uint32_t n, const float* rays, const int32_t* ignore, rgk_hit* hits, rgk_counters* counters) {
    if (!s || (!rays && n) || (!hits && n)) return fail(RGK_ERR_INVALID, "null argument");
    if (counters) std::memset(counters, 0, sizeof(*counters));
    if (n == 0) return RGK_OK;
    HIPCHK(hipSetDevice(s->device));
    int rc;
    if ((rc = ensure_workspace(s, n)) || (rc = s->nearfar.alloc(n)) || (rc = s->scratch_f.alloc((size_t)8 * n)) || (rc = s->scratch_u.alloc((size_t)5 * n)))
        return rc;
    hipStream_t st = s->stream;
    HIPCHK(hipMemcpyAsync(s->scratch_f.p, rays, (size_t)8 * n * sizeof(float), hipMemcpyHostToDevice, st));
    int32_t* d_ign = nullptr;
    if (ignore) {
        d_ign = (int32_t*)s->scratch_u.p;
        HIPCHK(hipMemcpyAsync(d_ign, ignore, (size_t)n * sizeof(int32_t), hipMemcpyHostToDevice, st));
    }
    HIPCHK(hipMemsetAsync(s->stats.p, 0, 8 * sizeof(unsigned long long), st));
    rgk_launch_init_counters(st, s->counters.p, n);
    rgk_launch_pack_rays(st, n, s->scratch_f.p, d_ign, s->rayA[0].p, s->rayB[0].p, s->nearfar.p);
    rgk_launch_set_bound(n, n);
    hipEvent_t e0 = nullptr, e1 = nullptr;
    if (counters) { HIPCHK(hipEventCreate(&e0)); HIPCHK(hipEventCreate(&e1)); HIPCHK(hipEventRecord(e0, st)); }
    rgk_launch_trace_closest(st, s->dev, s->tcfg, false, s->rayA[0].p, s->rayB[0].p, s->nearfar.p, s->hit.p,
                             s->counters.p + RGK_CNT_QUEUE, s->counters.p + RGK_CNT_FETCH_T, s->stats.p);
    if (counters) {
        HIPCHK(hipEventRecord(e1, st));
        rgk_launch_init_counters(st, s->counters.p, n);
        rgk_launch_trace_closest(st, s->dev, s->tcfg, true, s->rayA[0].p, s->rayB[0].p, s->nearfar.p, s->hit.p,
                                 s->counters.p + RGK_CNT_QUEUE, s->counters.p + RGK_CNT_FETCH_T, s->stats.p);
    }
    rgk_hit* d_hits = (rgk_hit*)s->scratch_u.p;
    rgk_launch_unpack_hits(st, n, s->hit.p, d_hits);
    HIPCHK(hipMemcpyAsync(hits, d_hits, (size_t)n * sizeof(rgk_hit), hipMemcpyDeviceToHost, st));
    HIPCHK(hipStreamSynchronize(st));
    HIPCHK(hipGetLastError());
    if (counters) {
        unsigned long long h[8];
        HIPCHK(hipMemcpy(h, s->stats.p, sizeof(h), hipMemcpyDeviceToHost));
        counters->node_visits = h[0]; counters->tri_tests = h[1]; counters->path_rays = n;
        if (s->tune.debug_util)
            std::fprintf(stderr, "[rgk util] rays %u  node visits %llu in %llu wave iterations (%.3f of lanes)  triangle tests %llu in %llu (%.3f)  outer iterations %llu  refills %llu\n",
// ... 120 lines not shown
```

rgk_amd/csrc/rgk_kernels.h:

```cpp
#pragma once
#include <hip/hip_runtime.h>
#include "device_types.h"

#ifndef RGK_TRACE_BLOCK
#define RGK_TRACE_BLOCK 256
#endif
#ifndef RGK_SHADE_WAVES
#define RGK_SHADE_WAVES 4
#endif
#ifndef RGK_SHADE_BLOCK
#define RGK_SHADE_BLOCK 512
#endif
#ifndef RGK_LIGHT_BLOCK
#define RGK_LIGHT_BLOCK RGK_SHADE_BLOCK
#endif
#ifndef RGK_SHADE_BLOCK_LATER
#define RGK_SHADE_BLOCK_LATER 256
#endif
#define RGK_MAX_DEPTH 62
#define RGK_LV_FLOAT4 6

#define RGK_CNT_QUEUE 0
#define RGK_CNT_SHADOW 64
#define RGK_CNT_FETCH_T 128
// ... 3 lines not shown
#define RGK_CNT_SRAYS 384
#define RGK_CNT_CONN 448
#define RGK_CNT_FETCH_J 512
#define RGK_CNT_TOTAL 576

#define RGK_SHADOW_ADD 0
#define RGK_SHADOW_SPLAT 2

#ifndef RGK_ENTRY_K
#define RGK_ENTRY_K 6
#endif
#ifndef RGK_ENTRY_SHIFT
#define RGK_ENTRY_SHIFT 3
#endif
#define RGK_ENTRY_PIX (1u << RGK_ENTRY_SHIFT)
struct PassParams {
    uint32_t j0, npix, s0, ns;
    uint32_t gshift;
    uint32_t beam;
    uint32_t multisample, depth, xres, yres;
    float clamp, russian, bumpmap_scale;
    uint32_t reverse;
    const uint32_t* pix_xy;
    const uint32_t* pix_seed;
    const float* htab;
    float4* light;
    const float4* lbox;
    const int* lentry;
    const float* entry_cap;
    const int* entry;
    float4* lstart;
    float4* lv;
    uint32_t* hitlist;
    uint32_t* lvmask;
    float4* conn;
    uint32_t* connlist;
    uint32_t batch;
    uint32_t* generic;
};

__device__ __forceinline__ void slot_decode(const PassParams& pp, uint32_t slot, uint32_t& j, uint32_t& srel) {
    const uint32_t r = slot >> pp.gshift, sb = r / pp.npix;
    j = r - sb * pp.npix;
    srel = (sb << pp.gshift) | (slot & ((1u << pp.gshift) - 1u));
}
__device__ __forceinline__ uint32_t slot_of(const PassParams& pp, uint32_t j, uint32_t srel) {
    return ((((srel >> pp.gshift) * pp.npix) + j) << pp.gshift) | (srel & ((1u << pp.gshift) - 1u));
}

void rgk_launch_entry_points(hipStream_t st, const DevScene& sc, const DevCamera& cam, uint32_t xres, uint32_t yres, const uint32_t* pix_xy, uint32_t n_pixels,
                             uint32_t g_first, uint32_t g_count, const uint32_t* trange, int* entries, float* cap);
void rgk_launch_group_trange(hipStream_t st, const PassParams& pp, const float4* hit, uint32_t* trange);
void rgk_launch_light_entry_points(hipStream_t st, const DevScene& sc, const DevCamera& cam, const PassParams& pp, uint32_t n_pixels_round, const uint32_t* trange, int* entries, float4* lbox);
void rgk_launch_stage_mark(hipStream_t st, uint32_t* host_word, uint32_t v);
void rgk_launch_init_counters(hipStream_t st, uint32_t* counters, uint32_t n0);
void rgk_launch_build_pixel_list(hipStream_t st, const rgk_tile* tiles, const uint32_t* tile_off, uint32_t n_tiles, uint32_t* pix_xy, uint32_t* pix_seed);
void rgk_launch_build_halton_table(hipStream_t st, const DevScene& sc, uint32_t S, float* htab);
struct RgkTraceCfg {
    int stack, lds;
    int* ovf;
};
int rgk_trace_grid(int lds_entries);
void rgk_launch_set_bound(uint32_t items, uint32_t shadow_items);
void rgk_launch_trace_camera(hipStream_t st, const DevScene& sc, const DevCamera& cam, const PassParams& pp, const RgkTraceCfg& tc, bool count_stats, float4* hit,
                             const uint32_t* count_ptr, uint32_t* fetch, unsigned long long* stats);
void rgk_launch_trace_closest(hipStream_t st, const DevScene& sc, const RgkTraceCfg& tc, bool count_stats, const float4* rayA, const float4* rayB,
                              const float2* nearfar, float4* hit, const uint32_t* count_ptr, uint32_t* fetch, unsigned long long* stats);
void rgk_launch_trace_shadow(hipStream_t st, const DevScene& sc, const RgkTraceCfg& tc, bool count_stats, const float4* shA, const float4* shB,
                             const float4* shC, float4* tot, uint8_t* vis_out, int mode, float* splat_rgb, const uint32_t* count_ptr,
                             uint32_t* fetch, unsigned long long* stats);
void rgk_launch_trace_shadow_first(hipStream_t st, const DevScene& sc, const PassParams& pp, const RgkTraceCfg& tc, bool count_stats, const float4* shA, const float4* shB,
                                   const float4* shC, float4* tot, const uint32_t* count_ptr, uint32_t* fetch, unsigned long long* stats);
void rgk_launch_raygen_light(hipStream_t st, const DevScene& sc, const DevCamera& cam, const PassParams& pp, float4* rayA, float4* rayB,
                             float4* thr, uint32_t* counters);
void rgk_launch_shade_light(hipStream_t st, const DevScene& sc, const DevCamera& cam, const PassParams& pp, uint32_t k, const float4* rayA,
                            const float4* rayB, const float4* hit, float4* thr, float4* nextA, float4* nextB, float4* shA, float4* shB,
                            float4* shC, uint32_t* counters);
void rgk_launch_list_hits(hipStream_t st, const float4* hit, const uint32_t* count_ptr, uint32_t* list, uint32_t* list_count);
void rgk_launch_connect(hipStream_t st, const DevScene& sc, const PassParams& pp, uint32_t bounce, float4* jobs, float4* rads, uint32_t* counters);
void rgk_launch_trace_shadow_jobs(hipStream_t st, const DevScene& sc, const PassParams& pp, const RgkTraceCfg& tc, bool count_stats, const float4* jobs, const float4* rads,
                                  float4* tot, const uint32_t* count_ptr, uint32_t* fetch, unsigned long long* stats);
void rgk_launch_shade(hipStream_t st, const DevScene& sc, const DevCamera& cam, const PassParams& pp, uint32_t bounce, const float4* rayA,
                      const float4* rayB, const float4* hit, float4* thr, float4* tot, float4* nextA, float4* nextB, float4* shA,
                      float4* shB, float4* shC, uint32_t* counters, bool bdpt = false);
void rgk_launch_resolve(hipStream_t st, const PassParams& pp, const float4* tot, float4* pixsum, float* accum_rgb, uint32_t* accum_count);
void rgk_launch_pack_rays(hipStream_t st, uint32_t n, const float* rays, const int32_t* ignore, float4* rayA, float4* rayB, float2* nearfar);
void rgk_launch_pack_visibility(hipStream_t st, const DevScene& sc, uint32_t n, const float* a, const float* b, float4* shA, float4* shB,
                                float4* shC);
void rgk_launch_unpack_hits(hipStream_t st, uint32_t n, const float4* hit, rgk_hit* out);
void rgk_launch_sampler_eval(hipStream_t st, const DevScene& sc, uint32_t n, const uint32_t* seed, const uint32_t* index,
                             const uint32_t* dim, int is2d, float* out);

void rgk_launch_bxdf_value(hipStream_t st, const DevScene& sc, uint32_t n, uint32_t route, const uint32_t* mat, const float* Vi, const float* Vr, const float* uv, float* out);
void rgk_launch_bxdf_sample(hipStream_t st, const DevScene& sc, uint32_t n, uint32_t route, const uint32_t* mat, const float* Vi, const float* uv, const float* u,
                            float* out_dir, float* out_w, uint8_t* leak);
void rgk_launch_texture_sample(hipStream_t st, const DevScene& sc, uint32_t n, const TexRef* refs, const int32_t* tex, const float* uv, float* rgb, float* sr, float* sb);
void rgk_launch_libm_eval(hipStream_t st, int fn, uint32_t n, const float* a, const float* b, float* out);
```

rgk_amd/csrc/rgk_kernels.hip:

```cpp
#include <hip/hip_runtime.h>
#include <cstdlib>
#include "rgk_device.h"
#include "rgk_kernels.h"

#ifndef RGK_TRANGE_ATOMIC
#define RGK_TRANGE_ATOMIC 0
#endif
#include "rgk_trace.h"

#ifndef RGK_SKIP_DEAD_NEE
#define RGK_SKIP_DEAD_NEE 1
#endif



template <bool GENERIC, bool FIRST, bool BDPT = false>
__global__ __launch_bounds__((FIRST ? RGK_SHADE_BLOCK : RGK_SHADE_BLOCK_LATER), RGK_SHADE_WAVES) void k_shade(const DevScene sc, const DevCamera cam, const PassParams pp, const uint32_t bounce,
                                                            const float4* __restrict__ rayA, const float4* __restrict__ rayB,
                                                            const float4* __restrict__ hit, float4* __restrict__ thr, float4* __restrict__ tot,
                                                            float4* __restrict__ nextA, float4* __restrict__ nextB, float4* __restrict__ shA,
                                                            float4* __restrict__ shB, float4* __restrict__ shC, uint32_t* __restrict__ counters) {
    const uint32_t count = counters[(GENERIC ? RGK_CNT_GENERIC : RGK_CNT_QUEUE) + bounce];
    const int lane = threadIdx.x & 63;
    const float eps = sc.epsilon;
    const SamplerTab tb = {pp.htab, pp.multisample};
    constexpr uint32_t BLK = FIRST ? RGK_SHADE_BLOCK : RGK_SHADE_BLOCK_LATER;
    __shared__ uint32_t s_cnt[4][BLK / 64];
    __shared__ uint32_t s_base[4];
    lut_lds_fill(sc);
    for (uint32_t base = blockIdx.x * BLK; base < count; base += gridDim.x * BLK) {
        const bool valid = base + threadIdx.x < count;
        const uint32_t i = !valid ? 0u : (GENERIC ? pp.generic[base + threadIdx.x] : base + threadIdx.x);
        bool cont = false, shadow = false, defer = false, conn = false;
        float4 nA = make_float4(0, 0, 0, 0), nB = nA, sA = nA, sB = nA, sC = nA;
        if (valid) {
            const float4 h = hit[i];
            uint32_t slot;
            f3 o, d;
            if (FIRST) { slot = i; camera_ray_of_slot(cam, pp, slot, o, d); }
            else {
                const float4 a = rayA[i], b = rayB[i];
                slot = __float_as_uint(b.w);
                o = mk3(a.x, a.y, a.z); d = mk3(a.w, b.x, b.y);
            }
            const float4 st = FIRST ? make_float4(1.f, 1.f, 1.f, __uint_as_float(1u << 16)) : thr[slot];
            const float4 li_slot = FIRST ? make_float4(0.f, 0.f, 0.f, 0.f) : pp.light[slot];
            f3 tot0 = mk3(0.f, 0.f, 0.f);
            float4 li_keep = make_float4(0.f, 0.f, 0.f, 0.f);
            f3 cum = mk3(st.x, st.y, st.z);
            uint32_t bits = __float_as_uint(st.w);
            uint32_t n = (bits & 0xffffu) + 1u;
            uint32_t c1 = bits >> 16;
            const int tri = __float_as_int(h.w);
            uint32_t srel, j; slot_decode(pp, slot, j, srel);
            const uint32_t seed = pp.pix_seed[pp.j0 + j];
            const uint32_t s = pp.s0 + srel;
            const uint32_t base2d = (cam.lens_size != 0.0f) ? 2u : 1u;
            const f3 Vr = -d;
            if (tri < 0) {
                f3 sky = skybox(sc, Vr);
                f3 add = cum * sky;
                if (FIRST && !GENERIC) tot0 = mk3(0.f + add.x, 0.f + add.y, 0.f + add.z);
                else {
                    float4 t = tot[slot];
                    t.x = t.x + add.x; t.y = t.y + add.y; t.z = t.z + add.z;
                    tot[slot] = t;
                }
            } else {
                const uint32_t tsr = (uint32_t)tri * (uint32_t)sizeof(TriShade);
                const float4 g0 = gld_f4(sc.tri_shade, tsr), g1 = gld_f4(sc.tri_shade, tsr + 16u), g2 = gld_f4(sc.tri_shade, tsr + 32u);
                const uint32_t mat_id = gld_u32(sc.tri_shade, tsr + 96u);
                const DevMaterial mat = mat_load(sc, mat_id);
                defer = !GENERIC && !mat_is_fast(mat.kind);
                if (!defer) {
                const float al = h.y, be = h.z;
                const float ia = 1.0f - al - be, ib = al, ic = be;
                f3 pos = o + h.x * d;
                f3 nA_ = mk3(g0.x, g0.y, g0.z), nB_ = mk3(g1.x, g1.y, g1.z), nC_ = mk3(g2.x, g2.y, g2.z);
                f3 faceN = ia * nA_ + ib * nB_ + ic * nC_;
                bool ok = true;
                if (faceN.x != faceN.x) {
                    faceN = nA_;
                    if (faceN.x != faceN.x) { faceN = nB_; if (faceN.x != faceN.x) { faceN = nC_; if (faceN.x != faceN.x) ok = false; } }
                }
                if (ok && len3(faceN) <= 0.0f) ok = false;
                if (ok) {
                    faceN = norm3(faceN);
                    const float4 g3 = gld_f4(sc.tri_shade, tsr + 48u), g4 = gld_f4(sc.tri_shade, tsr + 64u), g5 = gld_f4(sc.tri_shade, tsr + 80u);
                    float2 uv = make_float2(0.f, 0.f);
                    if (sc.has_texcoords) {
                        uv.x = ia * g0.w + ib * g2.w + ic * g4.w;
                        uv.y = ia * g1.w + ib * g3.w + ic * g5.w;
                    }
                    const bool bumped = tex_kind(mat.t_bump) != RGK_TEXREF_NONE;
                    f3 lightN = faceN;
                    if (bumped) {
                        float right, bottom;
                        tex_slopes(sc, mat.t_bump, uv, right, bottom);
                        f3 tangent = ia * mk3(g3.x, g3.y, g3.z) + ib * mk3(g4.x, g4.y, g4.z) + ic * mk3(g5.x, g5.y, g5.z);
                        if (!(tangent.x * tangent.x + tangent.y * tangent.y + tangent.z * tangent.z < 0.001f)) {
                            tangent = norm3(tangent);
                            f3 bitangent = norm3(cross3(faceN, tangent));
                            f3 tangent2 = cross3(bitangent, faceN);
                            lightN = norm3(faceN + (tangent2 * right + bitangent * bottom) * pp.bumpmap_scale);
                            if (lightN.x != lightN.x) lightN = faceN;
                        }
                    }
                    const quatf g2l = rotation_between(lightN, mk3(0.f, 0.f, 1.f));
                    const f3 VrL = qrot(g2l, Vr);
                    const bool last = !(n < pp.depth);
                    const bool no_russian = (mat.flags & RGK_MAT_NO_RUSSIAN) != 0;
                    const bool ends = last;
                    float4 li;
                    if (FIRST) {
                        f3 lpos;
                        const uint32_t lcode = light_code(sc, sample2d_t(tb, seed, s, base2d + 2u), sample1d_t(tb, seed, s, 0u), sample2d_t(tb, seed, s, base2d), lpos);
                        li = make_float4(lpos.x, lpos.y, lpos.z, __uint_as_float(lcode));
                    } else li = li_slot;
                    bool nee_dead = false;
                    if (RGK_SKIP_DEAD_NEE && ends && !GENERIC) {
                        const DLight L0 = light_from_code(sc, mk3(li.x, li.y, li.z), __float_as_uint(li.w));
                        if (L0.type < 0) nee_dead = true;
                        else {
                            const f3 df = pos - L0.pos;
                            nee_dead = dot3(df, df) > 0.f && (qrot(g2l, norm3(L0.pos - pos)).z <= 0.f || VrL.z <= 0.f);
                        }
                    }
                    MatPrep mp;
                    if (!nee_dead) mat_prepare(sc, mat, uv, VrL, !ends, mp);
                    else { mp.fast = true; mp.lobe = false; mp.diffc = mp.colorc = mk3(0.f, 0.f, 0.f); }
                    const f3 contribution = cum;
                    bool inside = false;
                    f3 dir = mk3(0.f, 0.f, 0.f);
                    uint32_t n_eff = n;
                    if (!ends) {
                        const quatf l2g = qinverse(g2l);
                        float2 u = sample2d_t(tb, seed, s, base2d + 3u + (n - 1u));
                        f3 dirL, weight; bool may_leak;
                        mat_sample<GENERIC>(sc, (int)mat_id, mat, mp, VrL, uv, u, dirL, weight, may_leak);
                        inside = dirL.z < 0;
                        dir = qrot(l2g, dirL);
                        if (!(dot3(dir, faceN) * dot3(Vr, faceN) > 0) && !may_leak) n_eff += 10000u;
                        const float rc = (!no_russian && pp.russian > 0.0f && n_eff > 1u) ? 1.0f / pp.russian : 1.0f;
                        cum = cum * rc;
                        cum = cum * weight;
                    }

                    {
                        li_keep = li;
                        const DLight L = light_from_code(sc, mk3(li.x, li.y, li.z), __float_as_uint(li.w));
                        f3 e_front = mk3(0.f, 0.f, 0.f);
                        if (dot3(faceN, Vr) > 0) e_front = mk3(mat.emission[0], mat.emission[1], mat.emission[2]);
                        const bool has_e = (e_front.x != 0.f) || (e_front.y != 0.f) || (e_front.z != 0.f);
                        if (BDPT) conn = ((pp.lvmask[slot] & 0x7fu) != 0u) || has_e;
                        f3 B = mk3(0.f, 0.f, 0.f);
                        if (has_e && !conn) {
                            B = clamp3(mk3(0.f, 0.f, 0.f) + e_front, pp.clamp) * contribution;
                            if (FIRST && !GENERIC) tot0 = mk3(0.f + B.x, 0.f + B.y, 0.f + B.z);
                            else {
                                float4 t = tot[slot];
                                t.x = t.x + B.x; t.y = t.y + B.y; t.z = t.z + B.z;
                                tot[slot] = t;
                            }
                        }
                        f3 out = mk3(0.f, 0.f, 0.f);
                        if (L.type >= 0 && !nee_dead) {
                            const f3 diff = pos - L.pos;
                            const f3 sd = norm3(diff);
                            const float slen = len3(diff);
                            const f3 Vi = norm3(L.pos - pos);
                            const f3 f = mat_value<GENERIC>(sc, (int)mat_id, mat, mp, qrot(g2l, Vi), VrL, uv);
                            const float G = fabsf(dot3(lightN, Vi)) / dot3(diff, diff);
                            const float k = L.intensity * light_dir_factor(L, -Vi);
                            const f3 inc = L.color * mk3(k, k, k);
                            out = inc * (f * G);
                            if (!conn) {
                                f3 A = clamp3((mk3(0.f, 0.f, 0.f) + out) + e_front, pp.clamp) * contribution;
                                f3 rad = has_e ? A - B : A;
                                if (rad.x != 0.f || rad.y != 0.f || rad.z != 0.f) {
                                    shadow = true;
                                    sA = make_float4(L.pos.x, L.pos.y, L.pos.z, sd.x);
                                    sB = make_float4(sd.y, sd.z, slen - eps * 20.0f, __uint_as_float(slot));
                                    sC = make_float4(rad.x, rad.y, rad.z, 0.0f + eps * 20.0f);
                                }
                            }
                        }
                        if (BDPT && conn) {
                            const size_t bs = pp.batch;
                            pp.conn[i] = make_float4(pos.x, pos.y, pos.z, __uint_as_float(slot));
                            pp.conn[bs + i] = make_float4(lightN.x, lightN.y, lightN.z, __uint_as_float(mat_id));
                            pp.conn[2 * bs + i] = make_float4(g2l.x, g2l.y, g2l.z, g2l.w);
                            pp.conn[3 * bs + i] = make_float4(VrL.x, VrL.y, VrL.z, uv.x);
                            pp.conn[4 * bs + i] = make_float4(contribution.x, contribution.y, contribution.z, uv.y);
                            pp.conn[5 * bs + i] = make_float4(out.x, out.y, out.z, __uint_as_float(has_e ? 1u : 0u));
                        }
                    }
                    bool go = !ends && !(max3c(cum) < 0.001f);
                    if (go && !no_russian && pp.russian >= 0.0f) {
                        float r = sample1d_t(tb, seed, s, c1);
                        c1++;
                        if (r > pp.russian) go = false;
                    }
                    if (go && n_eff > pp.depth) go = false;
                    if (go && !(n_eff < pp.depth)) go = false;
                    if (go) {
                        const float sgn = inside ? -1.0f : 1.0f;
                        f3 no = pos + faceN * eps * 10.0f * sgn;
                        f3 nd = norm3(norm3(dir));
                        cont = true;
                        nA = make_float4(no.x, no.y, no.z, nd.x);
                        nB = make_float4(nd.y, nd.z, __int_as_float(tri), __uint_as_float(slot));
                        thr[slot] = make_float4(cum.x, cum.y, cum.z, __uint_as_float((n & 0xffffu) | (c1 << 16)));
                    }
                    if (FIRST && (go || conn)) pp.light[slot] = li_keep;
                }
                }
            }
            if (FIRST && !GENERIC) tot[slot] = make_float4(tot0.x, tot0.y, tot0.z, 0.f);
        }
        {
            const unsigned long long m = __ballot(cont), ms = __ballot(shadow), md = __ballot(defer), mc = BDPT ? __ballot(conn) : 0ull;
            const int w = threadIdx.x >> 6;
            if (lane == 0) { s_cnt[0][w] = __popcll(m); s_cnt[1][w] = __popcll(ms); s_cnt[2][w] = __popcll(md); if (BDPT) s_cnt[3][w] = __popcll(mc); }
            __syncthreads();
            if (threadIdx.x == 0) {
                uint32_t t0 = 0, t1 = 0, t2 = 0, t3 = 0;
                for (int k = 0; k < (int)(BLK / 64); k++) {
                    uint32_t a = s_cnt[0][k], b = s_cnt[1][k], c = s_cnt[2][k];
                    s_cnt[0][k] = t0; s_cnt[1][k] = t1; s_cnt[2][k] = t2;
                    t0 += a; t1 += b; t2 += c;
                    if (BDPT) { uint32_t e = s_cnt[3][k]; s_cnt[3][k] = t3; t3 += e; }
                }
                s_base[0] = t0 ? atomicAdd(&counters[RGK_CNT_QUEUE + bounce + 1], t0) : 0u;
                s_base[1] = t1 ? atomicAdd(&counters[RGK_CNT_SHADOW + bounce], t1) : 0u;
                s_base[2] = t2 ? atomicAdd(&counters[RGK_CNT_GENERIC + bounce], t2) : 0u;
                if (BDPT) s_base[3] = t3 ? atomicAdd(&counters[RGK_CNT_CONN + bounce], t3) : 0u;
            }
            __syncthreads();
            if (!GENERIC && defer) pp.generic[s_base[2] + s_cnt[2][w] + __popcll(md & ((1ull << lane) - 1ull))] = i;
            if (BDPT && conn) pp.connlist[s_base[3] + s_cnt[3][w] + __popcll(mc & ((1ull << lane) - 1ull))] = i;
            if (cont) {
                uint32_t p = s_base[0] + s_cnt[0][w] + __popcll(m & ((1ull << lane) - 1ull));
                nextA[p] = nA; nextB[p] = nB;
            }
            if (shadow) {
                uint32_t p = s_base[1] + s_cnt[1][w] + __popcll(ms & ((1ull << lane) - 1ull));
                shA[p] = sA; shB[p] = sB; shC[p] = sC;
            }
            __syncthreads();
        }
    }
}

#include "rgk_bdpt.h"

__global__ __launch_bounds__(256) void k_resolve(const PassParams pp, const float4* __restrict__ tot, float4* __restrict__ pixsum,
                                                  float* __restrict__ accum_rgb, uint32_t* __restrict__ accum_count) {
    for (uint32_t j = blockIdx.x * blockDim.x + threadIdx.x; j < pp.npix; j += gridDim.x * blockDim.x) {
        float4 acc = (pp.s0 == 0) ? make_float4(0.f, 0.f, 0.f, 0.f) : pixsum[pp.j0 + j];
        for (uint32_t srel = 0; srel < pp.ns; srel++) {
            float4 t = tot[slot_of(pp, j, srel)];
            f3 v = clamp3(mk3(t.x, t.y, t.z), pp.clamp);
            if (v.x != v.x || v.x < 0.0f) v.x = 0.0f;
            if (v.y != v.y || v.y < 0.0f) v.y = 0.0f;
            if (v.z != v.z || v.z < 0.0f) v.z = 0.0f;
            acc.x = acc.x + v.x; acc.y = acc.y + v.y; acc.z = acc.z + v.z;
        }
        if (pp.s0 + pp.ns >= pp.multisample) {
            uint32_t pix = pp.pix_xy[pp.j0 + j];
            size_t p = (size_t)(pix >> 16) * pp.xres + (pix & 0xffff);
            accum_rgb[3 * p + 0] += acc.x;
            accum_rgb[3 * p + 1] += acc.y;
            accum_rgb[3 * p + 2] += acc.z;
            accum_count[p] += pp.multisample;
        } else {
            pixsum[pp.j0 + j] = acc;
        }
    }
}

__global__ __launch_bounds__(64) void k_resolve_tiled(const PassParams pp, const float4* __restrict__ tot, float4* __restrict__ pixsum,
                                                       float* __restrict__ accum_rgb, uint32_t* __restrict__ accum_count, const uint32_t PT) {
    extern __shared__ float4 tile[];
    const uint32_t G = 1u << pp.gshift, lane = threadIdx.x;
    for (uint32_t jb = blockIdx.x * PT; jb < pp.npix; jb += gridDim.x * PT) {
        const uint32_t np = min(PT, pp.npix - jb), j = jb + lane;
        float4 acc = make_float4(0.f, 0.f, 0.f, 0.f);
        if (lane < np && pp.s0 != 0) acc = pixsum[pp.j0 + j];
        for (uint32_t sb = 0; sb < (pp.ns >> pp.gshift); sb++) {
            const float4* __restrict__ src = tot + ((size_t)(sb * pp.npix + jb) << pp.gshift);
            for (uint32_t k = 0; k * 64u < np * G; k++) {
                const uint32_t idx = k * 64u + lane;
                if (idx < np * G) tile[(idx >> pp.gshift) * (G + 1u) + (idx & (G - 1u))] = src[idx];
            }
            __syncthreads();
            if (lane < np)
                for (uint32_t g = 0; g < G; g++) {
                    const float4 t = tile[lane * (G + 1u) + g];
                    f3 v = clamp3(mk3(t.x, t.y, t.z), pp.clamp);
                    if (v.x != v.x || v.x < 0.0f) v.x = 0.0f;
                    if (v.y != v.y || v.y < 0.0f) v.y = 0.0f;
                    if (v.z != v.z || v.z < 0.0f) v.z = 0.0f;
                    acc.x = acc.x + v.x; acc.y = acc.y + v.y; acc.z = acc.z + v.z;
                }
            __syncthreads();
        }
        if (lane < np) {
            if (pp.s0 + pp.ns >= pp.multisample) {
                uint32_t pix = pp.pix_xy[pp.j0 + j];
                size_t p = (size_t)(pix >> 16) * pp.xres + (pix & 0xffff);
                accum_rgb[3 * p + 0] += acc.x;
                accum_rgb[3 * p + 1] += acc.y;
                accum_rgb[3 * p + 2] += acc.z;
                accum_count[p] += pp.multisample;
            } else {
                pixsum[pp.j0 + j] = acc;
            }
        }
    }
}

__global__ __launch_bounds__(256) void k_build_pixel_list(const rgk_tile* __restrict__ tiles, const uint32_t* __restrict__ tile_off, uint32_t n_tiles,
                                                           uint32_t* __restrict__ pix_xy, uint32_t* __restrict__ pix_seed) {
    for (uint32_t t = blockIdx.x; t < n_tiles; t += gridDim.x) {
        const rgk_tile tl = tiles[t];
        const uint32_t tw = tl.x1 - tl.x0, th = tl.y1 - tl.y0, base = tile_off[t];
        for (uint32_t q = threadIdx.x; q < tw * th; q += blockDim.x) {
            const uint32_t nbr = (th + 7u) >> 3, nbc = (tw + 7u) >> 3;
            uint32_t r = q / (8u * tw);
            if (r > nbr - 1u) r = nbr - 1u;
// ... 327 lines not shown
    float amin = 1e30f, amax = -1e30f, bmin = 1e30f, bmax = -1e30f, wmax = 0.f, wmin = 1e30f;
    for (int k = 0; k < (rl > 0.f ? 16 : 8); k++) {
        const f3 q = k < 8 ? mk3((k & 1) ? bhi[0] : blo[0], (k & 2) ? bhi[1] : blo[1], (k & 4) ? bhi[2] : blo[2])
                           : mk3(lp.x + ((k & 1) ? rl : -rl), lp.y + ((k & 2) ? rl : -rl), lp.z + ((k & 4) ? rl : -rl));
        const f3 r = q - apex;
        const float rw = dot3(r, w);
        wmin = fminf(wmin, rw);
        if (k < 8) wmax = fmaxf(wmax, rw);
        if (rw > 0.f) { const float ra = dot3(r, u) / rw, rb = dot3(r, v) / rw; amin = fminf(amin, ra); amax = fmaxf(amax, ra); bmin = fminf(bmin, rb); bmax = fmaxf(bmax, rb); }
    }
    if (!(wmin > 0.02f * wmax)) return;
    const float am = 1e-4f * (1.f + fabsf(amin) + fabsf(amax)), bm = 1e-4f * (1.f + fabsf(bmin) + fabsf(bmax));
    amin -= am; amax += am; bmin -= bm; bmax += bm;
    f3 pl[5];
    float off[5] = {0.f, 0.f, 0.f, 0.f, 0.f};
    pl[0] = u - amin * w; pl[1] = amax * w - u; pl[2] = v - bmin * w; pl[3] = bmax * w - v;
    for (int k = 0; k < 4; k++) pl[k] = pl[k] * (1.0f / len3(pl[k]));
    pl[4] = -w; off[4] = -(wmax * 1.001f + pad);
    int list[RGK_ENTRY_K];
    entry_descent(sc, apex, pl, off, 5, pad, w, list);
    for (int k = 0; k < RGK_ENTRY_K; k++) e[k] = list[k];
    lbox[2 * (size_t)g] = make_float4(blo[0], blo[1], blo[2], 0.f);
    lbox[2 * (size_t)g + 1] = make_float4(bhi[0], bhi[1], bhi[2], 0.f);
}
void rgk_launch_entry_points(hipStream_t st, const DevScene& sc, const DevCamera& cam, uint32_t xres, uint32_t yres, const uint32_t* pix_xy, uint32_t n_pixels,
                             uint32_t g_first, uint32_t g_count, const uint32_t* trange, int* entries, float* cap) {
    k_entry_points<<<(g_count + 63u) / 64u, 64, 0, st>>>(sc, cam, xres, yres, pix_xy, n_pixels, g_first, g_count, trange, entries, cap);
}
void rgk_launch_group_trange(hipStream_t st, const PassParams& pp, const float4* hit, uint32_t* trange) {
    const uint32_t g_first = pp.j0 >> RGK_ENTRY_SHIFT, g_last = (pp.j0 + pp.npix + RGK_ENTRY_PIX - 1u) >> RGK_ENTRY_SHIFT, groups = g_last - g_first;
#if RGK_TRANGE_ATOMIC
    k_init_trange<<<(groups + 255u) / 256u, 256, 0, st>>>(trange + 2 * (size_t)g_first, groups);
    const uint32_t n = pp.npix * pp.ns;
    uint32_t blocks = (n + 255u) / 256u;
    if (blocks > 256u * 64u) blocks = 256u * 64u;
    k_group_trange<<<blocks, 256, 0, st>>>(pp, hit, n, trange);
#else
    k_group_trange_wave<<<groups, 64, 0, st>>>(pp, hit, g_first, groups, trange);
#endif
}
void rgk_launch_light_entry_points(hipStream_t st, const DevScene& sc, const DevCamera& cam, const PassParams& pp, uint32_t n_pixels_round, const uint32_t* trange, int* entries, float4* lbox) {
    const uint32_t g_first = pp.j0 >> RGK_ENTRY_SHIFT, g_last = (pp.j0 + pp.npix + RGK_ENTRY_PIX - 1u) >> RGK_ENTRY_SHIFT, groups = g_last - g_first;
    k_entry_points_light<<<(groups + 63u) / 64u, 64, 0, st>>>(sc, cam, pp.xres, pp.yres, pp.pix_xy, n_pixels_round, g_first, groups, trange, entries, lbox);
}

__global__ void k_stage_mark(uint32_t* host_word, uint32_t v) { *(volatile uint32_t*)host_word = v; __threadfence_system(); }
void rgk_launch_stage_mark(hipStream_t st, uint32_t* host_word, uint32_t v) { k_stage_mark<<<1, 1, 0, st>>>(host_word, v); }
void rgk_launch_init_counters(hipStream_t st, uint32_t* counters, uint32_t n0) { k_init_counters<<<1, 256, 0, st>>>(counters, n0); }
void rgk_launch_build_pixel_list(hipStream_t st, const rgk_tile* tiles, const uint32_t* tile_off, uint32_t n_tiles, uint32_t* pix_xy, uint32_t* pix_seed) {
    k_build_pixel_list<<<n_tiles < 4096u ? n_tiles : 4096u, 256, 0, st>>>(tiles, tile_off, n_tiles, pix_xy, pix_seed);
}
void rgk_launch_build_halton_table(hipStream_t st, const DevScene& sc, uint32_t S, float* htab) {
    uint32_t n = 192u * S;
    k_build_halton_table<<<(n + 255) / 256, 256, 0, st>>>(sc, S, htab);
}

void rgk_launch_trace_camera(hipStream_t st, const DevScene& sc, const DevCamera& cam, const PassParams& pp, const RgkTraceCfg& tc, bool count_stats, float4* hit,
                             const uint32_t* count_ptr, uint32_t* fetch, unsigned long long* stats) {
    if (pp.beam && pp.gshift == 3 && cam.lens_size == 0.0f && tc.lds < tc.stack) {
        const int grid = bounded_grid(rgk_trace_grid(tc.lds), (g_bound >> 3) + 1u, RGK_TRACE_BLOCK);
        if (count_stats) k_trace_camera_beam<true, 256, 8><<<grid, RGK_TRACE_BLOCK, 0, st>>>(sc, cam, pp, hit, count_ptr, fetch, stats, tc.ovf);
        else k_trace_camera_beam<false, 256, 8><<<grid, RGK_TRACE_BLOCK, 0, st>>>(sc, cam, pp, hit, count_ptr, fetch, stats, tc.ovf);
        return;
    }
    RGK_TRACE_DISPATCH(k_trace_camera, g_bound, sc, cam, pp, hit, count_ptr, fetch, stats, tc.ovf)
}

void rgk_launch_trace_closest(hipStream_t st, const DevScene& sc, const RgkTraceCfg& tc, bool count_stats, const float4* rayA, const float4* rayB,
                              const float2* nearfar, float4* hit, const uint32_t* count_ptr, uint32_t* fetch, unsigned long long* stats) {
    RGK_TRACE_DISPATCH(k_trace_closest, g_bound, sc, rayA, rayB, nearfar, hit, count_ptr, fetch, stats, tc.ovf)
}

void rgk_launch_trace_shadow(hipStream_t st, const DevScene& sc, const RgkTraceCfg& tc, bool count_stats, const float4* shA, const float4* shB,
                             const float4* shC, float4* tot, uint8_t* vis_out, int mode, float* splat_rgb, const uint32_t* count_ptr,
                             uint32_t* fetch, unsigned long long* stats) {
    RGK_TRACE_DISPATCH(k_trace_shadow, g_bound_shadow, sc, shA, shB, shC, tot, vis_out, mode, splat_rgb, count_ptr, fetch, stats, tc.ovf)
}

void rgk_launch_trace_shadow_first(hipStream_t st, const DevScene& sc, const PassParams& pp, const RgkTraceCfg& tc, bool count_stats, const float4* shA, const float4* shB,
                                   const float4* shC, float4* tot, const uint32_t* count_ptr, uint32_t* fetch, unsigned long long* stats) {
    RGK_TRACE_DISPATCH(k_trace_shadow_first, g_bound_shadow, sc, pp, shA, shB, shC, tot, count_ptr, fetch, stats, tc.ovf)
}

void rgk_launch_shade(hipStream_t st, const DevScene& sc, const DevCamera& cam, const PassParams& pp, uint32_t bounce, const float4* rayA,
                      const float4* rayB, const float4* hit, float4* thr, float4* tot, float4* nextA, float4* nextB, float4* shA,
                      float4* shB, float4* shC, uint32_t* counters, bool bdpt) {
    const int blk = bounce == 0 ? RGK_SHADE_BLOCK : RGK_SHADE_BLOCK_LATER;
    const int g1 = bounded_grid(256 * 4 * 512 / blk, g_bound, blk), g2 = bounded_grid(256 * 2 * 512 / blk, g_bound, blk);
    if (bdpt && bounce == 0) {
        k_shade<false, true, true><<<g1, blk, RGK_LDS_SHADE_BYTES, st>>>(sc, cam, pp, bounce, rayA, rayB, hit, thr, tot, nextA, nextB, shA, shB, shC, counters);
        k_shade<true, true, true><<<g2, blk, RGK_LDS_SHADE_BYTES, st>>>(sc, cam, pp, bounce, rayA, rayB, hit, thr, tot, nextA, nextB, shA, shB, shC, counters);
    } else if (bdpt) {
        k_shade<false, false, true><<<g1, blk, RGK_LDS_SHADE_BYTES, st>>>(sc, cam, pp, bounce, rayA, rayB, hit, thr, tot, nextA, nextB, shA, shB, shC, counters);
        k_shade<true, false, true><<<g2, blk, RGK_LDS_SHADE_BYTES, st>>>(sc, cam, pp, bounce, rayA, rayB, hit, thr, tot, nextA, nextB, shA, shB, shC, counters);
    } else if (bounce == 0) {
        k_shade<false, true><<<g1, blk, RGK_LDS_SHADE_BYTES, st>>>(sc, cam, pp, bounce, rayA, rayB, hit, thr, tot, nextA, nextB, shA, shB, shC, counters);
        k_shade<true, true><<<g2, blk, RGK_LDS_SHADE_BYTES, st>>>(sc, cam, pp, bounce, rayA, rayB, hit, thr, tot, nextA, nextB, shA, shB, shC, counters);
    } else {
        k_shade<false, false><<<g1, blk, RGK_LDS_SHADE_BYTES, st>>>(sc, cam, pp, bounce, rayA, rayB, hit, thr, tot, nextA, nextB, shA, shB, shC, counters);
        k_shade<true, false><<<g2, blk, RGK_LDS_SHADE_BYTES, st>>>(sc, cam, pp, bounce, rayA, rayB, hit, thr, tot, nextA, nextB, shA, shB, shC, counters);
    }
}

void rgk_launch_resolve(hipStream_t st, const PassParams& pp, const float4* tot, float4* pixsum, float* accum_rgb, uint32_t* accum_count) {
    int grid = (int)((pp.npix + 255) / 256);
    if (grid > 256 * 16) grid = 256 * 16;
    if (pp.gshift == 0) { k_resolve<<<grid, 256, 0, st>>>(pp, tot, pixsum, accum_rgb, accum_count); return; }
    const uint32_t G = 1u << pp.gshift;
    const uint32_t PT = G <= 8 ? 64u : 512u / G;
    int tiles = (int)((pp.npix + PT - 1) / PT);
    k_resolve_tiled<<<tiles > 256 * 64 ? 256 * 64 : tiles, 64, PT * (G + 1) * sizeof(float4), st>>>(pp, tot, pixsum, accum_rgb, accum_count, PT);
}

void rgk_launch_pack_rays(hipStream_t st, uint32_t n, const float* rays, const int32_t* ignore, float4* rayA, float4* rayB, float2* nearfar) {
    k_pack_rays<<<(n + 255) / 256, 256, 0, st>>>(n, rays, ignore, rayA, rayB, nearfar);
}
void rgk_launch_pack_visibility(hipStream_t st, const DevScene& sc, uint32_t n, const float* a, const float* b, float4* shA, float4* shB, float4* shC) {
    k_pack_visibility<<<(n + 255) / 256, 256, 0, st>>>(sc, n, a, b, shA, shB, shC);
}
void rgk_launch_unpack_hits(hipStream_t st, uint32_t n, const float4* hit, rgk_hit* out) { k_unpack_hits<<<(n + 255) / 256, 256, 0, st>>>(n, hit, out); }
void rgk_launch_sampler_eval(hipStream_t st, const DevScene& sc, uint32_t n, const uint32_t* seed, const uint32_t* index, const uint32_t* dim,
                             int is2d, float* out) {
    k_sampler_eval<<<(n + 255) / 256, 256, 0, st>>>(sc, n, seed, index, dim, is2d, out);
}

static inline int slot_grid(const PassParams& pp) {
    uint32_t n = pp.npix * pp.ns;
    int grid = (int)((n + 255) / 256);
    return grid > 256 * 16 ? 256 * 16 : grid;
}
void rgk_launch_raygen_light(hipStream_t st, const DevScene& sc, const DevCamera& cam, const PassParams& pp, float4* rayA, float4* rayB,
                             float4* thr, uint32_t* counters) {
    const uint32_t n = pp.npix * pp.ns;
    k_raygen_light<<<bounded_grid(256 * 4 * 512 / RGK_LIGHT_BLOCK, n, RGK_LIGHT_BLOCK), RGK_LIGHT_BLOCK, 0, st>>>(sc, cam, pp, rayA, rayB, thr, counters);
}
void rgk_launch_shade_light(hipStream_t st, const DevScene& sc, const DevCamera& cam, const PassParams& pp, uint32_t k, const float4* rayA,
                            const float4* rayB, const float4* hit, float4* thr, float4* nextA, float4* nextB, float4* shA, float4* shB,
                            float4* shC, uint32_t* counters) {
    k_shade_light<false><<<bounded_grid(256 * 4 * 512 / RGK_LIGHT_BLOCK, g_bound, RGK_LIGHT_BLOCK), RGK_LIGHT_BLOCK, RGK_LDS_SHADE_BYTES, st>>>(sc, cam, pp, k, rayA, rayB, hit, thr, nextA, nextB, shA, shB, shC, counters);
    k_shade_light<true><<<bounded_grid(256 * 2 * 512 / RGK_LIGHT_BLOCK, g_bound, RGK_LIGHT_BLOCK), RGK_LIGHT_BLOCK, RGK_LDS_SHADE_BYTES, st>>>(sc, cam, pp, k, rayA, rayB, hit, thr, nextA, nextB, shA, shB, shC, counters);
}
void rgk_launch_connect(hipStream_t st, const DevScene& sc, const PassParams& pp, uint32_t bounce, float4* jobs, float4* rads, uint32_t* counters) {
    k_connect<<<bounded_grid(256 * 8, g_bound, 256), 256, RGK_LDS_SHADE_BYTES, st>>>(sc, pp, bounce, jobs, rads, counters);
}
void rgk_launch_list_hits(hipStream_t st, const float4* hit, const uint32_t* count_ptr, uint32_t* list, uint32_t* list_count) {
    k_list_hits<<<bounded_grid(256 * 4 * 512 / RGK_LIGHT_BLOCK, g_bound, RGK_LIGHT_BLOCK), RGK_LIGHT_BLOCK, 0, st>>>(hit, count_ptr, list, list_count);
}
void rgk_launch_trace_shadow_jobs(hipStream_t st, const DevScene& sc, const PassParams& pp, const RgkTraceCfg& tc, bool count_stats, const float4* jobs, const float4* rads,
                                  float4* tot, const uint32_t* count_ptr, uint32_t* fetch, unsigned long long* stats) {
    RGK_TRACE_DISPATCH(k_trace_shadow_jobs, g_bound_shadow, sc, pp, jobs, rads, tot, count_ptr, fetch, stats, tc.ovf)
}
```

rgk_amd/csrc/rgk_trace.h:

```cpp
#pragma once
#include <hip/hip_runtime.h>
#include "rgk_device.h"
#include "rgk_kernels.h"

#define STACK_SENTINEL 0x7fffffff
#ifndef RGK_CHUNK_MAX
#define RGK_CHUNK_MAX 2048u
#endif
#ifndef RGK_TRACE_WAVES
#define RGK_TRACE_WAVES 8
#endif
#ifndef RGK_JOB_FINISH_ATOMIC
#define RGK_JOB_FINISH_ATOMIC 0
#endif
#ifndef RGK_JOB_REFILL_BELOW
#define RGK_JOB_REFILL_BELOW 24
#endif
#ifndef RGK_REFILL_BELOW_CAMERA
#define RGK_REFILL_BELOW_CAMERA 24
#endif
#ifndef RGK_REFILL_BELOW_ANY
#define RGK_REFILL_BELOW_ANY 24
#endif
#ifndef RGK_REFILL_BELOW
// ... 3 lines not shown
__device__ __forceinline__ void camera_ray(const DevCamera& cam, int x, int y, int xres, int yres, float2 off, float2 lens, f3& o, f3& d) {
    float fx = (x + off.x) / (float)(xres), fy = (y + off.y) / (float)(yres);
    f3 vs = mk3(cam.viewscreen[0], cam.viewscreen[1], cam.viewscreen[2]);
    f3 vx = mk3(cam.viewscreen_x[0], cam.viewscreen_x[1], cam.viewscreen_x[2]);
    f3 vy = mk3(cam.viewscreen_y[0], cam.viewscreen_y[1], cam.viewscreen_y[2]);
    f3 p = vs + fx * vx + fy * vy;
    o = mk3(cam.origin[0], cam.origin[1], cam.origin[2]);
    if (cam.lens_size != 0.0f) {
        float2 dsc = disc_uniform(lens);
        float lx = dsc.x * cam.lens_size, ly = dsc.y * cam.lens_size;
        o = o + lx * mk3(cam.left[0], cam.left[1], cam.left[2]) + ly * mk3(cam.up[0], cam.up[1], cam.up[2]);
    }
    d = norm3(p - o);
}
__device__ __forceinline__ void camera_ray_of_slot(const DevCamera& cam, const PassParams& pp, uint32_t slot, f3& o, f3& d, uint32_t* j_out = nullptr) {
    uint32_t srel, j; slot_decode(pp, slot, j, srel);
    if (j_out) *j_out = pp.j0 + j;
    const uint32_t pix = pp.pix_xy[pp.j0 + j], seed = pp.pix_seed[pp.j0 + j];
    const uint32_t s = pp.s0 + srel;
    const SamplerTab tb = {pp.htab, pp.multisample};
    const float2 jit = sample2d_t(tb, seed, s, 0);
    float2 lens = make_float2(0.f, 0.f);
    if (cam.lens_size != 0.0f) lens = sample2d_t(tb, seed, s, 1);
    camera_ray(cam, (int)(pix & 0xffff), (int)(pix >> 16), (int)pp.xres, (int)pp.yres, jit, lens, o, d);
}

__device__ __forceinline__ bool tri_test(const float4 r0, const float4 r1, const float4 r2, const f3 o, const f3 d,
                                         const float eps, float& t, float& alpha, float& beta) {
#if defined(RGK_DIAG_NO_TRI)
    t = r0.x + r1.x + r2.x + o.x + d.x; alpha = beta = 0.f;
    return t == 12345.678f;
#endif
    f3 n = mk3(r0.x, r0.y, r0.z);
    double dotv = (double)dot3(d, n);
    if (dotv != dotv) return false;
    if (dotv < (double)eps && dotv > (double)(-eps)) return false;
    double dot2 = (double)dot3(o, n);
    t = (float)(-((double)r0.w + dot2) / dotv);
    uint32_t axes = __float_as_uint(r2.z);
    int i1 = axes & 3, i2 = (axes >> 2) & 3;
    float px = comp(o, i1) + comp(d, i1) * t;
    float py = comp(o, i2) + comp(d, i2) * t;
    float q0x = px - r1.x, q0y = py - r1.y;
    float q1x = r1.z, q1y = r1.w, q2x = r2.x, q2y = r2.y;
    if (q1x > -eps && q1x < eps) {
        beta = q0x / q2x;
        if (beta < 0 || beta > 1) return false;
        alpha = (q0y - beta * q2y) / q1y;
    } else {
        beta = (q0y * q1x - q0x * q1y) / (q2y * q1x - q2x * q1y);
        if (beta < 0 || beta > 1) return false;
        alpha = (q0x - beta * q2x) / q1x;
    }
    if (alpha < 0 || (double)(alpha + beta) > 1.0) return false;
    return true;
}

__device__ __forceinline__ bool clip_to_scene(const DevScene& sc, f3 o, f3 d, float tnear, float tfar, float& t0, float& t1) {
    t0 = tnear; t1 = tfar;
    for (int i = 0; i < 3; ++i) {
        float invRayDir = 1.f / comp(d, i);
        float tN = (sc.bb_min[i] - comp(o, i)) * invRayDir;
        float tF = (sc.bb_max[i] - comp(o, i)) * invRayDir;
        if (tN > tF) { float s = tN; tN = tF; tF = s; }
        t0 = tN > t0 ? tN : t0;
        t1 = tF < t1 ? tF : t1;
        if (t0 > t1) return false;
    }
    return true;
}

__device__ __forceinline__ uint32_t fetch_chunk(uint32_t count, uint32_t nwaves, uint32_t pieces) {
    uint32_t c = (count / (nwaves * pieces)) & ~63u;
    return c < 64u ? 64u : (c > RGK_CHUNK_MAX ? RGK_CHUNK_MAX : c);
}

__device__ __forceinline__ float cvt_ubyte(uint32_t w, int c) { return (float)((w >> (8 * c)) & 0xffu); }

__device__ __forceinline__ int lds_pop(const int* p) {
    int v;
    asm volatile("ds_read_b32 %0, %1\n\ts_waitcnt lgkmcnt(0)" : "=v"(v) : "v"((uint32_t)(uintptr_t)p) : "memory");
    return v;
}
template <bool ANY, bool COUNT, int STACK, int LDSN, bool RAYGEN = false, bool JOB = false>
__device__ __forceinline__ void trace_persistent(const DevScene& sc, const float4* __restrict__ q0, const float4* __restrict__ q1,
                                                 const float4* __restrict__ q2, const float2* __restrict__ nearfar,
                                                 float4* __restrict__ hit, float4* __restrict__ tot, uint8_t* __restrict__ vis_out,
                                                 const int mode, float* __restrict__ splat_rgb,
                                                 const uint32_t count, uint32_t* __restrict__ fetch, int* __restrict__ stack, int* __restrict__ ovf, const uint32_t ostride,
                                                 uint32_t& n_nodes, uint32_t& n_tris, const DevCamera* cam = nullptr, const PassParams* pp = nullptr,
                                                 unsigned long long* __restrict__ util = nullptr) {
    const int lane = threadIdx.x & 63;
    uint32_t u_node_it = 0, u_leaf_it = 0, u_outer_it = 0, u_refill = 0;
    const int stride = RGK_TRACE_BLOCK;
    const float eps = sc.epsilon;
    const int walk_q = (int)sc.walk_q;
    const float4* __restrict__ nodes = reinterpret_cast<const float4*>(sc.nodes);
    const float4* __restrict__ tris = reinterpret_cast<const float4*>(sc.tris);
    const uint32_t chunk = fetch_chunk(count, gridDim.x * (RGK_TRACE_BLOCK / 64), ANY ? 4u : 16u);
    const uint32_t n_waves = gridDim.x * (RGK_TRACE_BLOCK / 64), wave_id = blockIdx.x * (RGK_TRACE_BLOCK / 64) + (threadIdx.x >> 6);
    uint32_t w_next = min(wave_id * chunk, count), w_end = min(w_next + chunk, count);
    bool exhausted = false;
    bool active = false;
    uint32_t idx = 0, ignore = 0xffffffffu, slot = 0;
    f3 o = mk3(0.f, 0.f, 0.f), d = o, inv = o, rad = o;
    float tlo = 0.f, thi = 0.f, best_t = 0.f, best_a = 0.f, best_b = 0.f;
    int best_tri = -1, cur = STACK_SENTINEL, sp = 0;
    f3 jsum = o;
    uint32_t jmask = 0;
    bool seg_pending = false;

#define RGK_PUT(x) { if (LDSN >= STACK || sp < LDSN) stack[sp * stride] = (x); else ovf[(size_t)(sp - LDSN) * ostride] = (x); }
#define RGK_JOB_RAY(from_, p_)                                                                                                         \
    {                                                                                                                                  \
        o = (from_);                                                                                                                   \
        const f3 diff_ = (p_) - o;                                                                                                     \
        d = norm3(diff_);                                                                                                              \
        const float tf_ = len3(diff_) - eps * 20.0f, tn_ = 0.0f + eps * 20.0f;                                                         \
        best_t = __builtin_inff(); best_tri = -1;                                                                                      \
        sp = 0;                                                                                                                        \
        float t0_, t1_;                                                                                                                \
        const bool nan_ = (o.x != o.x) | (o.y != o.y) | (o.z != o.z) | (d.x != d.x) | (d.y != d.y) | (d.z != d.z);                     \
        if (!nan_ && clip_to_scene(sc, o, d, tn_, tf_, t0_, t1_)) {                                                                    \
            tlo = t0_ - eps; thi = t1_ + eps;                                                                                          \
            inv = mk3(fminf(fmaxf(1.f / d.x, -1e30f), 1e30f), fminf(fmaxf(1.f / d.y, -1e30f), 1e30f), fminf(fmaxf(1.f / d.z, -1e30f), 1e30f)); \
            cur = 0;                                                                                                                   \
            seg_pending = false;                                                                                                       \
        } else jsum = jsum + rad;                                                                                                      \
    }
#if defined(RGK_POP_FLAT)
#define RGK_POP() ((LDSN >= STACK || sp < LDSN) ? stack[sp * stride] : ovf[(size_t)(sp - LDSN) * ostride])
#else
#define RGK_POP() ((LDSN >= STACK || sp < LDSN) ? lds_pop(stack + sp * stride) : ovf[(size_t)(sp - LDSN) * ostride])
#endif
    for (;;) {
        const unsigned long long occ = __ballot(active);
        unsigned long long act = JOB ? __ballot(active && !seg_pending) : occ;
        const int nact = __popcll(act);
        if (COUNT) u_outer_it++;
        const bool refill_now = nact <= (JOB ? RGK_JOB_REFILL_BELOW : RAYGEN ? RGK_REFILL_BELOW_CAMERA : ANY ? RGK_REFILL_BELOW_ANY : RGK_REFILL_BELOW);
        if (refill_now && !(exhausted && w_next >= w_end)) {
            if (COUNT) u_refill++;
            if (w_next >= w_end) {
                uint32_t base = 0;
                if (n_waves * chunk >= count) base = count;
                else if (lane == 0) base = atomicAdd(fetch, chunk) + n_waves * chunk;
                base = __builtin_amdgcn_readfirstlane(base);
                if (base >= count) exhausted = true;
                else { w_next = base; w_end = min(base + chunk, count); }
            }
            const uint32_t avail = (w_end > w_next) ? (w_end - w_next) : 0u;
            if (avail) {
                const unsigned long long idle = ~occ;
                const uint32_t rank = __popcll(idle & ((1ull << lane) - 1ull));
                if (!active && rank < avail) {
                    idx = w_next + rank;
                    float tn = 0.0f, tf = 10000.0f;
                    uint32_t pixel_j = 0;
                    if (JOB) {
                        const float4 a = q0[idx], f0 = q0[3 * (size_t)pp->batch + idx], r0 = q1[idx];
                        jmask = __float_as_uint(q0[(size_t)pp->batch + idx].w);
                        jsum = mk3(0.f, 0.f, 0.f);
                        ignore = 0xffffffffu;
                        cur = STACK_SENTINEL; sp = 0;
                        seg_pending = true; active = true;
                        if (jmask & 1u) {
                            jmask &= ~1u;
                            rad = mk3(r0.x, r0.y, r0.z);
                            RGK_JOB_RAY(mk3(f0.x, f0.y, f0.z), mk3(a.x, a.y, a.z))
                        }
                    } else
                    if (RAYGEN) {
                        camera_ray_of_slot(*cam, *pp, idx, o, d, &pixel_j);
                        ignore = 0xffffffffu;
                    } else {
                        const float4 a = q0[idx], b = q1[idx];
                        o = mk3(a.x, a.y, a.z); d = mk3(a.w, b.x, b.y);
                        if (ANY) {
                            const float4 c = q2[idx];
                            rad = mk3(c.x, c.y, c.z); tn = c.w; tf = b.z;
                            slot = __float_as_uint(b.w);
                            ignore = 0xffffffffu;
                        } else {
                            ignore = __float_as_uint(b.z);
                            if (nearfar) { float2 nf = nearfar[idx]; tn = nf.x; tf = nf.y; }
                        }
                    }
                    if (!JOB) {
                    best_t = __builtin_inff(); best_tri = -1; best_a = 0.f; best_b = 0.f;
                    float t0, t1;
                    sp = 0;
                    const bool nan_ray = (o.x != o.x) | (o.y != o.y) | (o.z != o.z) | (d.x != d.x) | (d.y != d.y) | (d.z != d.z);
                    if (!nan_ray && clip_to_scene(sc, o, d, tn, tf, t0, t1)) {
                        tlo = t0 - eps; thi = t1 + eps;
                        inv = mk3(fminf(fmaxf(1.f / d.x, -1e30f), 1e30f), fminf(fmaxf(1.f / d.y, -1e30f), 1e30f), fminf(fmaxf(1.f / d.z, -1e30f), 1e30f));
                        cur = 0;
                        if (ANY && pp && pp->lentry) {
                            uint32_t srel, j;
                            slot_decode(*pp, slot, j, srel);
                            const size_t grp = (size_t)((pp->j0 + j) >> RGK_ENTRY_SHIFT);
                            const float4 blo = pp->lbox[2 * grp], bhi = pp->lbox[2 * grp + 1];
                            const f3 end = o + tf * d;
                            if (end.x >= blo.x && end.x <= bhi.x && end.y >= blo.y && end.y <= bhi.y && end.z >= blo.z && end.z <= bhi.z) {
                                const int* e = pp->lentry + grp * RGK_ENTRY_K;
                                cur = e[0];
#pragma unroll
                                for (int k = RGK_ENTRY_K - 1; k >= 1; k--) { const int r = e[k]; if (r != STACK_SENTINEL) { RGK_PUT(r) sp++; } }
                            }
                        }
                        if (RAYGEN && pp->entry) {
                            const float capd = pp->entry_cap[pixel_j >> RGK_ENTRY_SHIFT];
                            if (capd < thi) { thi = capd; ignore = 0xfffffffeu; }
                            const int* e = pp->entry + (size_t)(pixel_j >> RGK_ENTRY_SHIFT) * RGK_ENTRY_K;
                            cur = e[0];
#pragma unroll
                            for (int k = RGK_ENTRY_K - 1; k >= 1; k--) { const int r = e[k]; if (r != STACK_SENTINEL) { RGK_PUT(r) sp++; } }
                        }
                    } else cur = STACK_SENTINEL;
                    active = true;
                    }
                }
                const uint32_t taken = min(avail, (uint32_t)(64 - __popcll(occ)));
                w_next += taken;
            }
            act = __ballot(active);
        }
        if (JOB && refill_now) {
            while (active && seg_pending) {
                const float4 a = q0[idx];
                const uint32_t jslot = __float_as_uint(a.w);
                const uint32_t m = jmask & 0xffu;
                if (m == 0u) {
                    f3 total = jsum;
                    if (jmask & 0x100u) { const float4 e = q0[2 * (size_t)pp->batch + idx]; total = total + mk3(e.x, e.y, e.z); }
                    total = clamp3(total, pp->clamp);
                    const float4 c = q0[(size_t)pp->batch + idx];
                    const f3 add = total * mk3(c.x, c.y, c.z);
#if RGK_JOB_FINISH_ATOMIC
                    float* tp = reinterpret_cast<float*>(tot + jslot);
                    unsafeAtomicAdd(tp, add.x); unsafeAtomicAdd(tp + 1, add.y); unsafeAtomicAdd(tp + 2, add.z);
#else
                    float4 t = tot[jslot];
                    t.x = t.x + add.x; t.y = t.y + add.y; t.z = t.z + add.z;
                    tot[jslot] = t;
#endif
                    active = false; seg_pending = false;
                    break;
                }
                const uint32_t q = (uint32_t)__builtin_ctz(m);
                jmask &= ~(1u << q);
                const float4 r = q1[(size_t)q * pp->batch + idx];
                rad = mk3(r.x, r.y, r.z);
                const float4 fr = (q == 0u) ? q0[3 * (size_t)pp->batch + idx] : pp->lv[(size_t)((q - 1u) * RGK_LV_FLOAT4) * pp->batch + jslot];
                RGK_JOB_RAY(mk3(fr.x, fr.y, fr.z), mk3(a.x, a.y, a.z))
            }
            act = __ballot(active);
// ... 308 lines not shown
                if (mx == 2u) { t0x = -__builtin_inff(); t1x = __builtin_inff(); }
                if (my == 2u) { t0y = -__builtin_inff(); t1y = __builtin_inff(); }
                if (mz == 2u) { t0z = -__builtin_inff(); t1z = __builtin_inff(); }
                const float tn = fmaxf(fmaxf(fmaxf(t0x, t0y), t0z), btlo);
                const float tf = fminf(fminf(fminf(t1x, t1y), t1z), limit);
                const bool h = (ref[c] != STACK_SENTINEL) && (tn <= tf);
                te[c] = h ? tn : __builtin_inff();
                if (!h) ref[c] = STACK_SENTINEL;
            }
#define RGK_CSWAP(a, b) { const bool sw = te[b] < te[a]; const float tt = sw ? te[b] : te[a], tu = sw ? te[a] : te[b]; \
                          const int rr = sw ? ref[b] : ref[a], ru = sw ? ref[a] : ref[b]; te[a] = tt; te[b] = tu; ref[a] = rr; ref[b] = ru; }
            RGK_CSWAP(0, 1) RGK_CSWAP(2, 3) RGK_CSWAP(0, 2) RGK_CSWAP(1, 3) RGK_CSWAP(1, 2)
#undef RGK_CSWAP
            RGK_PUT(ref[3]) sp += (ref[3] != STACK_SENTINEL);
            RGK_PUT(ref[2]) sp += (ref[2] != STACK_SENTINEL);
            RGK_PUT(ref[1]) sp += (ref[1] != STACK_SENTINEL);
            cur = ref[0];
            if (cur == STACK_SENTINEL && sp > 0) { sp--; cur = RGK_POP(); }
        }
        if (active && cur < 0) {
            const uint32_t code = ~(uint32_t)cur;
            const uint32_t first = code >> 4, cnt = (code & 15u) + 1u;
            for (uint32_t k = 0; k < cnt; k++) {
                const float4 r0 = tris[3 * (first + k) + 0], r1 = tris[3 * (first + k) + 1], r2 = tris[3 * (first + k) + 2];
                const int tid = (int)__float_as_uint(r2.w);
                if (COUNT) n_tris += (uint32_t)__popc(valid);
                for (int q = 0; q < 8; q++) {
                    if (!(valid & (1u << q))) continue;
                    const f3 dq = RGK_D(q);
                    float t, al, be;
                    if (!tri_test(r0, r1, r2, o, dq, eps, t, al, be)) continue;
                    float t0, t1;
                    (void)clip_to_scene(sc, o, dq, 0.0f, 10000.0f, t0, t1);
                    const float thi = capped ? fminf(t1 + eps, capd) : t1 + eps;
                    if (t < t0 - eps || t > thi) continue;
                    const float bq = RGK_BEST(q);
                    bool take = t < bq;
                    if (t == bq) take = tid > __float_as_int(hit[((size_t)idx << 3) + q].w);
                    if (take) { RGK_BEST(q) = t; hit[((size_t)idx << 3) + q] = make_float4(t, al, be, __int_as_float(tid)); }
                }
            }
            bmax = 0.f;
            for (int q = 0; q < 8; q++) if (valid & (1u << q)) bmax = fmaxf(bmax, RGK_BEST(q));
            if (sp > 0) { sp--; cur = RGK_POP(); }
            else cur = STACK_SENTINEL;
        }
        if (active && cur == STACK_SENTINEL) {
            uint32_t again = 0;
            if (capped) {
                for (int q = 0; q < 8; q++) if ((valid & (1u << q)) && RGK_BEST(q) == __builtin_inff()) again |= 1u << q;
            }
            if (again) {
                valid = again; capped = false; capd = __builtin_inff(); bmax = __builtin_inff();
                RGK_BEAM_BOUNDS()
                cur = 0; sp = 0;
            } else active = false;
        }
    }
#undef RGK_BEAM_BOUNDS
#undef RGK_D
#undef RGK_BEST
    if (COUNT) {
        atomicAdd(&stats[0], (unsigned long long)n_nodes);
        atomicAdd(&stats[1], (unsigned long long)n_tris);
    }
}

template <bool COUNT, int STACK, int LDSN>
__global__ __launch_bounds__(RGK_TRACE_BLOCK, (LDSN <= 16 ? RGK_TRACE_WAVES : 5)) void k_trace_shadow(const DevScene sc, const float4* __restrict__ shA,
                                                                   const float4* __restrict__ shB, const float4* __restrict__ shC,
                                                                   float4* __restrict__ tot, uint8_t* __restrict__ vis_out,
                                                                   const int mode, float* __restrict__ splat_rgb,
                                                                   const uint32_t* __restrict__ count_ptr, uint32_t* __restrict__ fetch,
                                                                   unsigned long long* __restrict__ stats, int* __restrict__ ovf) {
    __shared__ int lds_stack[LDSN * RGK_TRACE_BLOCK];
    uint32_t n_nodes = 0, n_tris = 0;
    trace_persistent<true, COUNT, STACK, LDSN>(sc, shA, shB, shC, nullptr, nullptr, tot, vis_out, mode, splat_rgb, *count_ptr, fetch,
                                         lds_stack + threadIdx.x, ovf + (blockIdx.x * RGK_TRACE_BLOCK + threadIdx.x), gridDim.x * RGK_TRACE_BLOCK, n_nodes, n_tris);
    if (COUNT) {
        atomicAdd(&stats[2], (unsigned long long)n_nodes);
        atomicAdd(&stats[3], (unsigned long long)n_tris);
    }
}

#ifndef RGK_JOB_FINISH_ATOMIC
#define RGK_JOB_FINISH_ATOMIC 0
#endif
#ifndef RGK_JOB_WAVES
#define RGK_JOB_WAVES 6
#endif
template <bool COUNT, int STACK, int LDSN>
__global__ __launch_bounds__(RGK_TRACE_BLOCK, (LDSN <= 16 ? RGK_JOB_WAVES : 5)) void k_trace_shadow_jobs(const DevScene sc, const PassParams pp, const float4* __restrict__ jobs,
                                                                   const float4* __restrict__ rads, float4* __restrict__ tot,
                                                                   const uint32_t* __restrict__ count_ptr, uint32_t* __restrict__ fetch,
                                                                   unsigned long long* __restrict__ stats, int* __restrict__ ovf) {
    __shared__ int lds_stack[LDSN * RGK_TRACE_BLOCK];
    uint32_t n_nodes = 0, n_tris = 0;
    trace_persistent<true, COUNT, STACK, LDSN, false, true>(sc, jobs, rads, nullptr, nullptr, nullptr, tot, nullptr, RGK_SHADOW_ADD, nullptr, *count_ptr, fetch,
                                         lds_stack + threadIdx.x, ovf + (blockIdx.x * RGK_TRACE_BLOCK + threadIdx.x), gridDim.x * RGK_TRACE_BLOCK, n_nodes, n_tris, nullptr, &pp);
    if (COUNT) {
        atomicAdd(&stats[2], (unsigned long long)n_nodes);
        atomicAdd(&stats[3], (unsigned long long)n_tris);
    }
}

template <bool COUNT, int STACK, int LDSN>
__global__ __launch_bounds__(RGK_TRACE_BLOCK, (LDSN <= 16 ? RGK_TRACE_WAVES : 5)) void k_trace_shadow_first(const DevScene sc, const PassParams pp, const float4* __restrict__ shA,
                                                                   const float4* __restrict__ shB, const float4* __restrict__ shC,
                                                                   float4* __restrict__ tot, const uint32_t* __restrict__ count_ptr, uint32_t* __restrict__ fetch,
                                                                   unsigned long long* __restrict__ stats, int* __restrict__ ovf) {
    __shared__ int lds_stack[LDSN * RGK_TRACE_BLOCK];
    uint32_t n_nodes = 0, n_tris = 0;
    trace_persistent<true, COUNT, STACK, LDSN>(sc, shA, shB, shC, nullptr, nullptr, tot, nullptr, RGK_SHADOW_ADD, nullptr, *count_ptr, fetch,
                                         lds_stack + threadIdx.x, ovf + (blockIdx.x * RGK_TRACE_BLOCK + threadIdx.x), gridDim.x * RGK_TRACE_BLOCK, n_nodes, n_tris, nullptr, &pp);
    if (COUNT) {
        atomicAdd(&stats[2], (unsigned long long)n_nodes);
        atomicAdd(&stats[3], (unsigned long long)n_tris);
    }
}
```

Baseline: 4473 Mpaths/s.

## Specialize single point-light scenes with compact 32-byte shadow records

Detects scenes with exactly one zero-size point light, where host-side float checks show light selection is deterministic. For those scenes, shading and shadow tracing are specialised: the light position comes from scene constants instead of per-path light sampling and the pp.light buffer, and shadow records shrink from three float4 to two by dropping the light origin and tmin. This cuts sampling arithmetic and global memory traffic in shade and shadow kernels, at the cost of extra kernel instantiations and an eligibility check that must exactly reproduce the generic light choice.

```diff
diff --git a/include/rgk.h b/include/rgk.h
--- a/include/rgk.h
+++ b/include/rgk.h
@@ -203,6 +203,7 @@
     uint32_t n_leaf_refs;
     uint32_t n_float_textures;
     uint32_t n_palettized_textures;
+    uint32_t const_light;
 } rgk_scene_info;
 
 typedef struct rgk_hit {
diff --git a/rgk_amd/capi.py b/rgk_amd/capi.py
--- a/rgk_amd/capi.py
+++ b/rgk_amd/capi.py
@@ -104,7 +104,8 @@
                 ("total_areal_power", C.c_float), ("total_point_power", C.c_float),
                 ("n_nodes", C.c_uint32), ("node_bytes", C.c_uint32), ("tri_bytes", C.c_uint32),
                 ("max_depth", C.c_uint32), ("n_leaf_refs", C.c_uint32),
-                ("n_float_textures", C.c_uint32), ("n_palettized_textures", C.c_uint32)]
+                ("n_float_textures", C.c_uint32), ("n_palettized_textures", C.c_uint32),
+                ("const_light", C.c_uint32)]
 
 
 class Progress(C.Structure):
diff --git a/rgk_amd/csrc/device_types.h b/rgk_amd/csrc/device_types.h
--- a/rgk_amd/csrc/device_types.h
+++ b/rgk_amd/csrc/device_types.h
@@ -115,6 +115,7 @@
     const uint16_t* hperm;
     uint32_t n_pointlights, n_areal;
     float total_point_power, total_areal_power;
+    float cl_pos[3], cl_intensity, cl_color[3];
     float epsilon;
     float bb_min[3], bb_max[3];
     uint32_t has_texcoords;
diff --git a/rgk_amd/csrc/rgk_device.h b/rgk_amd/csrc/rgk_device.h
--- a/rgk_amd/csrc/rgk_device.h
+++ b/rgk_amd/csrc/rgk_device.h
@@ -713,6 +713,15 @@
     L.intensity = pl->intensity; L.size = pl->size;
     return L;
 }
+__device__ __forceinline__ DLight light_constant(const DevScene& sc) {
+    DLight L;
+    L.pos = mk3(sc.cl_pos[0], sc.cl_pos[1], sc.cl_pos[2]);
+    L.color = mk3(sc.cl_color[0], sc.cl_color[1], sc.cl_color[2]);
+    L.normal = mk3(0.f, 0.f, 0.f);
+    L.intensity = sc.cl_intensity; L.size = 0.f; L.index = 0;
+    L.type = 0;
+    return L;
+}
 __device__ __forceinline__ f3 skybox(const DevScene& sc, f3 direction) {
     if (sc.sky_mode == 0) return mk3(sc.sky_color[0], sc.sky_color[1], sc.sky_color[2]) * mk3(sc.sky_intensity, sc.sky_intensity, sc.sky_intensity);
     float alpha = rgk_asinf(direction.y);
diff --git a/rgk_amd/csrc/rgk_host.cpp b/rgk_amd/csrc/rgk_host.cpp
--- a/rgk_amd/csrc/rgk_host.cpp
+++ b/rgk_amd/csrc/rgk_host.cpp
@@ -453,12 +453,32 @@
     bool entry_points = true;
     bool entry_cap = true;
     bool light_entry = true;
+    bool const_light = true;
     int sample_group = -1;
     size_t batch_paths = 0;
     double workspace_gb = 0;
     int beam = 1;
     bool debug_bvh = false, debug_util = false;
 };
+
+static uint32_t const_light_eligible(const DevScene& ds, const DevPointLight* pls) {
+    if (ds.n_pointlights != 1 || ds.n_areal != 0) return 0;
+    const DevPointLight& pl = pls[0];
+    if (pl.size != 0.0f) return 0;
+    for (int k = 0; k < 3; k++)
+        if (pl.pos[k] == 0.0f && std::signbit(pl.pos[k])) return 0;
+    const float PI_F = 3.14159265358979323846264338327950288f;
+    volatile float total_power = ds.total_point_power + ds.total_areal_power;
+    if (total_power <= 0.0f) return 0;
+    const float choice_max = 0x1.fffffep-1f;
+    volatile float q = choice_max * total_power;
+    if (!(q < ds.total_point_power)) return 0;
+    volatile float step = pl.intensity * 4.0f;
+    step = step * PI_F;
+    q = q - step;
+    if (!(q <= 0.0f)) return 0;
+    return 1;
+}
 
 struct rgk_scene {
     int device = 0;
@@ -476,6 +496,7 @@
     DevBuf<uint32_t> texels8;
     DevBuf<float> luts;
     DevBuf<DevPointLight> pointlights;
+    DevPointLight h_light0{};
     DevBuf<DevArealLight> areal;
     DevBuf<DevArealTri> areal_tris;
     DevBuf<float4> ltc;
@@ -773,6 +794,7 @@
         auto off = [](const char* name) { const char* e = std::getenv(name); return e && e[0] == '0'; };
         RgkTuning& t = s->tune;
         t.entry_points = !off("RGK_ENTRY_POINTS"); t.entry_cap = !off("RGK_ENTRY_CAP"); t.light_entry = !off("RGK_LIGHT_ENTRY");
+        t.const_light = !off("RGK_CONST_LIGHT");
         if (const char* e = std::getenv("RGK_SAMPLE_GROUP")) t.sample_group = std::min(6, std::max(0, std::atoi(e)));
         if (const char* e = std::getenv("RGK_BATCH_PATHS")) t.batch_paths = std::max<size_t>(1024, strtoull(e, nullptr, 10));
         if (const char* e = std::getenv("RGK_WORKSPACE_GB")) t.workspace_gb = atof(e);
@@ -1113,6 +1135,11 @@
     ds.ltc = s->ltc.p; ds.hdims = s->hdims.p; ds.hperm = s->hperm.p;
     ds.n_pointlights = (uint32_t)pls.size(); ds.n_areal = (uint32_t)als.size();
     ds.total_point_power = total_point; ds.total_areal_power = total_areal;
+    if (!pls.empty()) {
+        s->h_light0 = pls[0];
+        for (int k = 0; k < 3; k++) { ds.cl_pos[k] = pls[0].pos[k]; ds.cl_color[k] = pls[0].color[k]; }
+        ds.cl_intensity = pls[0].intensity;
+    }
     ds.has_texcoords = d->texcoords ? 1u : 0u;
     ds.sky_mode = d->sky_mode;
     for (int k = 0; k < 3; k++) ds.sky_color[k] = d->sky_color[k];
@@ -1128,6 +1155,7 @@
     inf.n_nodes = n_nodes; inf.node_bytes = RGK_NODE_BYTES; inf.tri_bytes = RGK_TRI_BYTES;
     inf.max_depth = max_depth; inf.n_leaf_refs = n_refs;
     inf.n_float_textures = n_float_tex; inf.n_palettized_textures = n_palettized;
+    inf.const_light = const_light_eligible(ds, &s->h_light0);
     guard.s = nullptr;
     *out = s;
     return RGK_OK;
@@ -1170,6 +1198,7 @@
     for (int a = 0; a < 3; a++) { ds.bb_min[a] = mn[a] - eps; ds.bb_max[a] = mx[a] + eps; }
     if (hipMemcpy(s->self.p, &ds, sizeof(DevScene), hipMemcpyHostToDevice) != hipSuccess) return fail(RGK_ERR_DEVICE, "hipMemcpy(DevScene)");
     s->info.epsilon = eps; s->info.total_areal_power = total_areal;
+    s->info.const_light = const_light_eligible(ds, &s->h_light0);
     for (int a = 0; a < 3; a++) { s->info.bbox_min[a] = ds.bb_min[a]; s->info.bbox_max[a] = ds.bb_max[a]; }
     s->entry_key = 0; s->entry_n = 0; s->entry_capped = 0; s->lentry_done = 0;
     return RGK_OK;
@@ -1199,6 +1228,7 @@
     if (k == "entry_points") t.entry_points = value != 0;
     else if (k == "entry_cap") t.entry_cap = value != 0;
     else if (k == "light_entry") t.light_entry = value != 0;
+    else if (k == "const_light") t.const_light = value != 0;
     else if (k == "sample_group") t.sample_group = value < 0 ? -1 : (int)std::min(6.0, value);
     else if (k == "batch_paths") t.batch_paths = value <= 0 ? 0 : std::max<size_t>(1024, (size_t)value);
     else if (k == "workspace_gb") t.workspace_gb = value <= 0 ? 0.0 : value;
@@ -1462,7 +1492,7 @@
     return 0;
 }
 
-int queue_pass(rgk_scene* s, KernelLog& kl, const DevCamera& cam, PassParams& pp, size_t P, bool light_entry, float* d_accum_rgb,
+int queue_pass(rgk_scene* s, KernelLog& kl, const DevCamera& cam, PassParams& pp, size_t P, bool light_entry, bool const_light, float* d_accum_rgb,
                uint32_t* d_accum_count, uint32_t stage) {
     hipStream_t st = s->stream;
     const RgkTraceCfg& tc = s->tcfg;
@@ -1507,10 +1537,14 @@
         else
             rc = kl.run(RGK_K_TRACE_CLOSEST, [&] { rgk_launch_trace_closest(st, s->dev, tc, count_stats, rayA[q], rayB[q], nullptr, hit, cn + RGK_CNT_QUEUE + b, cn + RGK_CNT_FETCH_T + b, s->stats.p); });
         if (rc || (b == 0 && (rc = queue_first_hit_lists(s, kl, cam, pp, (uint32_t)P, cap_entries, light_entry)))) return rc;
-        if ((rc = kl.run(b == 0 ? RGK_K_SHADE_FIRST : RGK_K_SHADE, [&] { rgk_launch_shade(st, s->dev, cam, pp, b, rayA[q], rayB[q], hit, thr, tot, rayA[q ^ 1], rayB[q ^ 1], shA, shB, shC, cn, R > 0); })) ||
+        if ((rc = kl.run(b == 0 ? RGK_K_SHADE_FIRST : RGK_K_SHADE, [&] { rgk_launch_shade(st, s->dev, cam, pp, b, rayA[q], rayB[q], hit, thr, tot, rayA[q ^ 1], rayB[q ^ 1], shA, shB, shC, cn, R > 0, const_light); })) ||
             (R > 0 && (rc = kl.run(RGK_K_CONNECT, [&] { rgk_launch_connect(st, s->dev, pp, b, s->jobs.p, s->rads.p, cn); }))))
             return rc;
-        if (b == 0 && light_entry)
+        if (const_light && rgk_const_light_records() && b == 0 && light_entry)
+            rc = kl.run(RGK_K_SHADOW_FIRST, [&] { rgk_launch_trace_shadow_first_cl(st, s->dev, pp, tc, count_stats, shA, shB, tot, cn + RGK_CNT_SHADOW + b, cn + RGK_CNT_FETCH_S + b, s->stats.p); });
+        else if (const_light && rgk_const_light_records())
+            rc = kl.run(RGK_K_SHADOW, [&] { rgk_launch_trace_shadow_cl(st, s->dev, tc, count_stats, shA, shB, tot, cn + RGK_CNT_SHADOW + b, cn + RGK_CNT_FETCH_S + b, s->stats.p); });
+        else if (b == 0 && light_entry)
             rc = kl.run(RGK_K_SHADOW_FIRST, [&] { rgk_launch_trace_shadow_first(st, s->dev, pp, tc, count_stats, shA, shB, shC, tot, cn + RGK_CNT_SHADOW + b, cn + RGK_CNT_FETCH_S + b, s->stats.p); });
         else
             rc = kl.run(RGK_K_SHADOW, [&] { rgk_launch_trace_shadow(st, s->dev, tc, count_stats, shA, shB, shC, tot, nullptr, RGK_SHADOW_ADD, nullptr, cn + RGK_CNT_SHADOW + b, cn + RGK_CNT_FETCH_S + b, s->stats.p); });
@@ -1567,6 +1601,7 @@
     pp.entry = s->entry.p;
     pp.entry_cap = s->entry_cap.p;
     const bool light_entry = s->entry.p && s->tune.light_entry && s->dev.n_pointlights == 1 && s->dev.n_areal == 0;
+    const bool const_light = s->info.const_light == 1 && s->tune.const_light && R == 0;
     if (light_entry) {
         const size_t groups = ((size_t)P + RGK_ENTRY_PIX - 1) / RGK_ENTRY_PIX + 1;
         if ((rc = s->lentry.alloc(groups * RGK_ENTRY_K)) || (rc = s->trange.alloc(groups * 2)) || (rc = s->lbox.alloc(groups * 2))) return rc;
@@ -1583,7 +1618,7 @@
         for (uint32_t s0 = 0; s0 < prm->multisample; s0 += ns_pass, stage += pass_stages) {
             pp.s0 = s0;
             pp.ns = std::min(ns_pass, prm->multisample - s0);
-            if ((rc = queue_pass(s, kl, cam, pp, P, light_entry, d_accum_rgb, d_accum_count, stage))) return rc;
+            if ((rc = queue_pass(s, kl, cam, pp, P, light_entry, const_light, d_accum_rgb, d_accum_count, stage))) return rc;
             HIPCHK(hipStreamSynchronize(s->stream));
             add_pass_counters(s->h_counters, pp, light_entry, tot);
         }
diff --git a/rgk_amd/csrc/rgk_kernels.h b/rgk_amd/csrc/rgk_kernels.h
--- a/rgk_amd/csrc/rgk_kernels.h
+++ b/rgk_amd/csrc/rgk_kernels.h
@@ -109,7 +109,12 @@
                                   float4* tot, const uint32_t* count_ptr, uint32_t* fetch, unsigned long long* stats);
 void rgk_launch_shade(hipStream_t st, const DevScene& sc, const DevCamera& cam, const PassParams& pp, uint32_t bounce, const float4* rayA,
                       const float4* rayB, const float4* hit, float4* thr, float4* tot, float4* nextA, float4* nextB, float4* shA,
-                      float4* shB, float4* shC, uint32_t* counters, bool bdpt = false);
+                      float4* shB, float4* shC, uint32_t* counters, bool bdpt = false, bool const_light = false);
+bool rgk_const_light_records();
+void rgk_launch_trace_shadow_cl(hipStream_t st, const DevScene& sc, const RgkTraceCfg& tc, bool count_stats, const float4* shA, const float4* shB,
+                                float4* tot, const uint32_t* count_ptr, uint32_t* fetch, unsigned long long* stats);
+void rgk_launch_trace_shadow_first_cl(hipStream_t st, const DevScene& sc, const PassParams& pp, const RgkTraceCfg& tc, bool count_stats, const float4* shA, const float4* shB,
+                                      float4* tot, const uint32_t* count_ptr, uint32_t* fetch, unsigned long long* stats);
 void rgk_launch_resolve(hipStream_t st, const PassParams& pp, const float4* tot, float4* pixsum, float* accum_rgb, uint32_t* accum_count);
 void rgk_launch_pack_rays(hipStream_t st, uint32_t n, const float* rays, const int32_t* ignore, float4* rayA, float4* rayB, float2* nearfar);
 void rgk_launch_pack_visibility(hipStream_t st, const DevScene& sc, uint32_t n, const float* a, const float* b, float4* shA, float4* shB,
diff --git a/rgk_amd/csrc/rgk_kernels.hip b/rgk_amd/csrc/rgk_kernels.hip
--- a/rgk_amd/csrc/rgk_kernels.hip
+++ b/rgk_amd/csrc/rgk_kernels.hip
@@ -11,10 +11,13 @@
 #ifndef RGK_SKIP_DEAD_NEE
 #define RGK_SKIP_DEAD_NEE 1
 #endif
-
-
-
-template <bool GENERIC, bool FIRST, bool BDPT = false>
+#ifndef RGK_CL_REC32
+#define RGK_CL_REC32 1
+#endif
+
+
+
+template <bool GENERIC, bool FIRST, bool BDPT = false, bool CL = false>
 __global__ __launch_bounds__((FIRST ? RGK_SHADE_BLOCK : RGK_SHADE_BLOCK_LATER), RGK_SHADE_WAVES) void k_shade(const DevScene sc, const DevCamera cam, const PassParams pp, const uint32_t bounce,
                                                             const float4* __restrict__ rayA, const float4* __restrict__ rayB,
                                                             const float4* __restrict__ hit, float4* __restrict__ thr, float4* __restrict__ tot,
@@ -44,7 +47,7 @@
                 o = mk3(a.x, a.y, a.z); d = mk3(a.w, b.x, b.y);
             }
             const float4 st = FIRST ? make_float4(1.f, 1.f, 1.f, __uint_as_float(1u << 16)) : thr[slot];
-            const float4 li_slot = FIRST ? make_float4(0.f, 0.f, 0.f, 0.f) : pp.light[slot];
+            const float4 li_slot = (FIRST || CL) ? make_float4(0.f, 0.f, 0.f, 0.f) : pp.light[slot];
             f3 tot0 = mk3(0.f, 0.f, 0.f);
             float4 li_keep = make_float4(0.f, 0.f, 0.f, 0.f);
             f3 cum = mk3(st.x, st.y, st.z);
@@ -112,14 +115,15 @@
                     const bool no_russian = (mat.flags & RGK_MAT_NO_RUSSIAN) != 0;
                     const bool ends = last;
                     float4 li;
-                    if (FIRST) {
+                    if (CL) li = make_float4(sc.cl_pos[0], sc.cl_pos[1], sc.cl_pos[2], __uint_as_float(0u));
+                    else if (FIRST) {
                         f3 lpos;
                         const uint32_t lcode = light_code(sc, sample2d_t(tb, seed, s, base2d + 2u), sample1d_t(tb, seed, s, 0u), sample2d_t(tb, seed, s, base2d), lpos);
                         li = make_float4(lpos.x, lpos.y, lpos.z, __uint_as_float(lcode));
                     } else li = li_slot;
                     bool nee_dead = false;
                     if (RGK_SKIP_DEAD_NEE && ends && !GENERIC) {
-                        const DLight L0 = light_from_code(sc, mk3(li.x, li.y, li.z), __float_as_uint(li.w));
+                        const DLight L0 = CL ? light_constant(sc) : light_from_code(sc, mk3(li.x, li.y, li.z), __float_as_uint(li.w));
                         if (L0.type < 0) nee_dead = true;
                         else {
                             const f3 df = pos - L0.pos;
@@ -148,7 +152,7 @@
 
                     {
                         li_keep = li;
-                        const DLight L = light_from_code(sc, mk3(li.x, li.y, li.z), __float_as_uint(li.w));
+                        const DLight L = CL ? light_constant(sc) : light_from_code(sc, mk3(li.x, li.y, li.z), __float_as_uint(li.w));
                         f3 e_front = mk3(0.f, 0.f, 0.f);
                         if (dot3(faceN, Vr) > 0) e_front = mk3(mat.emission[0], mat.emission[1], mat.emission[2]);
                         const bool has_e = (e_front.x != 0.f) || (e_front.y != 0.f) || (e_front.z != 0.f);
@@ -179,9 +183,14 @@
                                 f3 rad = has_e ? A - B : A;
                                 if (rad.x != 0.f || rad.y != 0.f || rad.z != 0.f) {
                                     shadow = true;
-                                    sA = make_float4(L.pos.x, L.pos.y, L.pos.z, sd.x);
-                                    sB = make_float4(sd.y, sd.z, slen - eps * 20.0f, __uint_as_float(slot));
-                                    sC = make_float4(rad.x, rad.y, rad.z, 0.0f + eps * 20.0f);
+                                    if (CL && RGK_CL_REC32) {
+                                        sA = make_float4(sd.x, sd.y, sd.z, slen - eps * 20.0f);
+                                        sB = make_float4(rad.x, rad.y, rad.z, __uint_as_float(slot));
+                                    } else {
+                                        sA = make_float4(L.pos.x, L.pos.y, L.pos.z, sd.x);
+                                        sB = make_float4(sd.y, sd.z, slen - eps * 20.0f, __uint_as_float(slot));
+                                        sC = make_float4(rad.x, rad.y, rad.z, 0.0f + eps * 20.0f);
+                                    }
                                 }
                             }
                         }
@@ -212,7 +221,7 @@
                         nB = make_float4(nd.y, nd.z, __int_as_float(tri), __uint_as_float(slot));
                         thr[slot] = make_float4(cum.x, cum.y, cum.z, __uint_as_float((n & 0xffffu) | (c1 << 16)));
                     }
-                    if (FIRST && (go || conn)) pp.light[slot] = li_keep;
+                    if (FIRST && !CL && (go || conn)) pp.light[slot] = li_keep;
                 }
                 }
             }
@@ -245,7 +254,8 @@
             }
             if (shadow) {
                 uint32_t p = s_base[1] + s_cnt[1][w] + __popcll(ms & ((1ull << lane) - 1ull));
-                shA[p] = sA; shB[p] = sB; shC[p] = sC;
+                shA[p] = sA; shB[p] = sB;
+                if (!(CL && RGK_CL_REC32)) shC[p] = sC;
             }
             __syncthreads();
         }
@@ -739,9 +749,19 @@
     RGK_TRACE_DISPATCH(k_trace_shadow_first, g_bound_shadow, sc, pp, shA, shB, shC, tot, count_ptr, fetch, stats, tc.ovf)
 }
 
+bool rgk_const_light_records() { return RGK_CL_REC32 != 0; }
+void rgk_launch_trace_shadow_cl(hipStream_t st, const DevScene& sc, const RgkTraceCfg& tc, bool count_stats, const float4* shA, const float4* shB,
+                                float4* tot, const uint32_t* count_ptr, uint32_t* fetch, unsigned long long* stats) {
+    RGK_TRACE_DISPATCH(k_trace_shadow_cl, g_bound_shadow, sc, shA, shB, tot, count_ptr, fetch, stats, tc.ovf)
+}
+void rgk_launch_trace_shadow_first_cl(hipStream_t st, const DevScene& sc, const PassParams& pp, const RgkTraceCfg& tc, bool count_stats, const float4* shA, const float4* shB,
+                                      float4* tot, const uint32_t* count_ptr, uint32_t* fetch, unsigned long long* stats) {
+    RGK_TRACE_DISPATCH(k_trace_shadow_first_cl, g_bound_shadow, sc, pp, shA, shB, tot, count_ptr, fetch, stats, tc.ovf)
+}
+
 void rgk_launch_shade(hipStream_t st, const DevScene& sc, const DevCamera& cam, const PassParams& pp, uint32_t bounce, const float4* rayA,
                       const float4* rayB, const float4* hit, float4* thr, float4* tot, float4* nextA, float4* nextB, float4* shA,
-                      float4* shB, float4* shC, uint32_t* counters, bool bdpt) {
+                      float4* shB, float4* shC, uint32_t* counters, bool bdpt, bool const_light) {
     const int blk = bounce == 0 ? RGK_SHADE_BLOCK : RGK_SHADE_BLOCK_LATER;
     const int g1 = bounded_grid(256 * 4 * 512 / blk, g_bound, blk), g2 = bounded_grid(256 * 2 * 512 / blk, g_bound, blk);
     if (bdpt && bounce == 0) {
@@ -750,6 +770,12 @@
     } else if (bdpt) {
         k_shade<false, false, true><<<g1, blk, RGK_LDS_SHADE_BYTES, st>>>(sc, cam, pp, bounce, rayA, rayB, hit, thr, tot, nextA, nextB, shA, shB, shC, counters);
         k_shade<true, false, true><<<g2, blk, RGK_LDS_SHADE_BYTES, st>>>(sc, cam, pp, bounce, rayA, rayB, hit, thr, tot, nextA, nextB, shA, shB, shC, counters);
+    } else if (const_light && bounce == 0) {
+        k_shade<false, true, false, true><<<g1, blk, RGK_LDS_SHADE_BYTES, st>>>(sc, cam, pp, bounce, rayA, rayB, hit, thr, tot, nextA, nextB, shA, shB, shC, counters);
+        k_shade<true, true, false, true><<<g2, blk, RGK_LDS_SHADE_BYTES, st>>>(sc, cam, pp, bounce, rayA, rayB, hit, thr, tot, nextA, nextB, shA, shB, shC, counters);
+    } else if (const_light) {
+        k_shade<false, false, false, true><<<g1, blk, RGK_LDS_SHADE_BYTES, st>>>(sc, cam, pp, bounce, rayA, rayB, hit, thr, tot, nextA, nextB, shA, shB, shC, counters);
+        k_shade<true, false, false, true><<<g2, blk, RGK_LDS_SHADE_BYTES, st>>>(sc, cam, pp, bounce, rayA, rayB, hit, thr, tot, nextA, nextB, shA, shB, shC, counters);
     } else if (bounce == 0) {
         k_shade<false, true><<<g1, blk, RGK_LDS_SHADE_BYTES, st>>>(sc, cam, pp, bounce, rayA, rayB, hit, thr, tot, nextA, nextB, shA, shB, shC, counters);
         k_shade<true, true><<<g2, blk, RGK_LDS_SHADE_BYTES, st>>>(sc, cam, pp, bounce, rayA, rayB, hit, thr, tot, nextA, nextB, shA, shB, shC, counters);
diff --git a/rgk_amd/csrc/rgk_trace.h b/rgk_amd/csrc/rgk_trace.h
--- a/rgk_amd/csrc/rgk_trace.h
+++ b/rgk_amd/csrc/rgk_trace.h
@@ -109,7 +109,7 @@
     asm volatile("ds_read_b32 %0, %1\n\ts_waitcnt lgkmcnt(0)" : "=v"(v) : "v"((uint32_t)(uintptr_t)p) : "memory");
     return v;
 }
-template <bool ANY, bool COUNT, int STACK, int LDSN, bool RAYGEN = false, bool JOB = false>
+template <bool ANY, bool COUNT, int STACK, int LDSN, bool RAYGEN = false, bool JOB = false, bool CLO = false>
 __device__ __forceinline__ void trace_persistent(const DevScene& sc, const float4* __restrict__ q0, const float4* __restrict__ q1,
                                                  const float4* __restrict__ q2, const float2* __restrict__ nearfar,
                                                  float4* __restrict__ hit, float4* __restrict__ tot, uint8_t* __restrict__ vis_out,
@@ -199,6 +199,14 @@
                     } else
                     if (RAYGEN) {
                         camera_ray_of_slot(*cam, *pp, idx, o, d, &pixel_j);
+                        ignore = 0xffffffffu;
+                    } else if (CLO) {
+                        const float4 a = q0[idx], b = q1[idx];
+                        o = mk3(sc.cl_pos[0], sc.cl_pos[1], sc.cl_pos[2]);
+                        d = mk3(a.x, a.y, a.z); tf = a.w;
+                        rad = mk3(b.x, b.y, b.z); slot = __float_as_uint(b.w);
+                        tn = 0.0f + eps * 20.0f;
+                        asm volatile("" : "+v"(o.x), "+v"(o.y), "+v"(o.z), "+v"(tn));
                         ignore = 0xffffffffu;
                     } else {
                         const float4 a = q0[idx], b = q1[idx];
@@ -673,6 +681,20 @@
         atomicAdd(&stats[3], (unsigned long long)n_tris);
     }
 }
+template <bool COUNT, int STACK, int LDSN>
+__global__ __launch_bounds__(RGK_TRACE_BLOCK, (LDSN <= 16 ? RGK_TRACE_WAVES : 5)) void k_trace_shadow_cl(const DevScene sc, const float4* __restrict__ shA,
+                                                                   const float4* __restrict__ shB, float4* __restrict__ tot,
+                                                                   const uint32_t* __restrict__ count_ptr, uint32_t* __restrict__ fetch,
+                                                                   unsigned long long* __restrict__ stats, int* __restrict__ ovf) {
+    __shared__ int lds_stack[LDSN * RGK_TRACE_BLOCK];
+    uint32_t n_nodes = 0, n_tris = 0;
+    trace_persistent<true, COUNT, STACK, LDSN, false, false, true>(sc, shA, shB, nullptr, nullptr, nullptr, tot, nullptr, RGK_SHADOW_ADD, nullptr, *count_ptr, fetch,
+                                         lds_stack + threadIdx.x, ovf + (blockIdx.x * RGK_TRACE_BLOCK + threadIdx.x), gridDim.x * RGK_TRACE_BLOCK, n_nodes, n_tris);
+    if (COUNT) {
+        atomicAdd(&stats[2], (unsigned long long)n_nodes);
+        atomicAdd(&stats[3], (unsigned long long)n_tris);
+    }
+}
 
 #ifndef RGK_JOB_FINISH_ATOMIC
 #define RGK_JOB_FINISH_ATOMIC 0
@@ -709,3 +731,18 @@
         atomicAdd(&stats[3], (unsigned long long)n_tris);
     }
 }
+
+template <bool COUNT, int STACK, int LDSN>
+__global__ __launch_bounds__(RGK_TRACE_BLOCK, (LDSN <= 16 ? RGK_TRACE_WAVES : 5)) void k_trace_shadow_first_cl(const DevScene sc, const PassParams pp, const float4* __restrict__ shA,
+                                                                   const float4* __restrict__ shB, float4* __restrict__ tot,
+                                                                   const uint32_t* __restrict__ count_ptr, uint32_t* __restrict__ fetch,
+                                                                   unsigned long long* __restrict__ stats, int* __restrict__ ovf) {
+    __shared__ int lds_stack[LDSN * RGK_TRACE_BLOCK];
+    uint32_t n_nodes = 0, n_tris = 0;
+    trace_persistent<true, COUNT, STACK, LDSN, false, false, true>(sc, shA, shB, nullptr, nullptr, nullptr, tot, nullptr, RGK_SHADOW_ADD, nullptr, *count_ptr, fetch,
+                                         lds_stack + threadIdx.x, ovf + (blockIdx.x * RGK_TRACE_BLOCK + threadIdx.x), gridDim.x * RGK_TRACE_BLOCK, n_nodes, n_tris, nullptr, &pp);
+    if (COUNT) {
+        atomicAdd(&stats[2], (unsigned long long)n_nodes);
+        atomicAdd(&stats[3], (unsigned long long)n_tris);
+    }
+}
```

Result: faster. 4716 Mpaths/s (median of 6 runs) (+5.4%).
